# Gadersd/whisper-burn

Hardware: AMD Instinct MI355X
Metric: real-time factor (audio-sec/wall-sec) (higher is better)
Workload: dtype f32; 1 GPU; tiny.en, 30 s of 16 kHz audio per GPU per step, reference windowing (3 windows <= 14.9 s, 3 s overlap), HIP mel + encoder + KV-cached decode, greedy (beam_size 1), max_depth 100; windows=3, beam_size=1, max_depth=100, encoder_gemm_after_the_run=f16x3, parallelism=windows sharded over 1 GPU(s), 1 token all-gather

## Files before the change

### whisper-burn_amd/csrc/decode.h

```cpp
#pragma once
#include <hip/hip_runtime.h>
#include <hip/hip_ext.h>
#include <stdint.h>

#include <algorithm>

#include "kernels.h"
#include "wb_internal.h"

namespace wb {

constexpr int MAX_BEAMS = 8;
constexpr int TOPK_MAX = 8;
constexpr int CA_STRIDE = 66;
constexpr int CA_NCH_MAX = 12;
constexpr int TS_STRIDE = 2 + 2 * TOPK_MAX;
constexpr int GV_CT = 128;
constexpr int GV_CT_LOGITS = 128;
constexpr int KS_MAX = 16;

enum { ST_N = 0, ST_STEP = 1, ST_HDR = 4 };
enum { GC_STEP = 0, GC_NDONE = 1, GC_ALLDONE = 2, GC_BAD = 3, GC_HDR = 4 };
struct StepLayout {
  int S = 0, W = 0;
  int tok = 0, parent = 0, len = 0, win = 0;
  int dead = 0;
  int win_nb = 0, win_slots = 0;
  int total = 0;
};
inline StepLayout make_step_layout(int S, int W) {
  StepLayout l;
  l.S = S; l.W = W;
  l.tok = ST_HDR; l.parent = l.tok + S; l.len = l.parent + S; l.win = l.len + S; l.dead = l.win + S;
  l.win_nb = l.dead + S; l.win_slots = l.win_nb + W; l.total = l.win_slots + W * MAX_BEAMS;
  return l;
}

enum { PRO_PLAIN = 0, PRO_GELU = 1, PRO_ATTN = 2, PRO_LN = 3 };
struct GemvArgs {
  const float* W = nullptr; int ldw = 0;
  int K = 0, N = 0, KS = 1, KSL = 0;
  int pro = PRO_PLAIN;
  const float* src = nullptr; int ld_src = 0;
  const float* pend = nullptr; const float* pbias = nullptr; int KSp = 0;
  float* x_out = nullptr;
  const float* ln_g = nullptr; const float* ln_b = nullptr; float ln_eps = 0.f; int ln_inside = 0;
  int n_head = 0, n_chunks = 0;
  float* P = nullptr;
  float* h_tmp = nullptr;
  const float* mask = nullptr; int use_mask = 0, topk = 0; float* tstats = nullptr;
  const int* st = nullptr; int S = 0;
  int ct = 0;
};

void gemv_plan(int K, int N, int* KS, int* KSL);
int cross_attn_chunk();

void launch_dec_prepare(hipStream_t st, const int* state_host_mapped, int* state_dev, const StepLayout& lay, int n,
                        int* tabs, int Lmax, const float* E, const float* pos, int d, float* x, const int* gctl);
void launch_dec_resolve_ln(hipStream_t st, const int* state, int n_max, const float* x_in, float* x_out,
                           const float* P, int KS, int S, const float* bias, int d, const LayerNormW& ln,
                           int eps_inside_sqrt, float* h);
void launch_dec_gemv(hipStream_t st, const GemvArgs& a, int n_rows_hint, bool stats);
bool dec_logits_two_launches(const GemvArgs& a, int n_rows_hint);
void launch_dec_self_attn(hipStream_t st, const int* state, const StepLayout& lay, int n_max, int n_head,
                          const float* Pqkv, int KS, const float* bqkv, int d, float* Kc, float* Vc, const int* tab,
                          int Lmax, float scale, float* att);
struct CaFuse {
  const float* x_in = nullptr;
  const float* pend = nullptr; int KSp = 0; const float* pbias = nullptr;
  float* x_out = nullptr;
  const float* ln_g = nullptr; const float* ln_b = nullptr; float ln_eps = 0.f; int ln_inside = 0;
  const float* Wq = nullptr;
  const float* Wo = nullptr;
  float* rec = nullptr;
};
bool cross_attn_can_fuse_q(int d);
void launch_dec_cross_attn(hipStream_t st, const int* state, const StepLayout& lay, int n_windows, int n_head,
                           int n_chunks, const float* Pq, int KS, const float* bq, int d, const float* ckv, int ldkv,
                           int koff, const int* win_row0, const int* win_C, float scale, float* ca, int max_nb,
                           const CaFuse* fuse = nullptr);
constexpr int CSF_MAX_D = 1280;
struct CaStreamFuse {
  const float* x_in = nullptr; float* x_out = nullptr;
  const float* pend = nullptr; int KSp = 0; const float* pbias = nullptr;
  const float* ln_g = nullptr; const float* ln_b = nullptr; float ln_eps = 0.f; int ln_inside = 0;
  const float* Wq = nullptr;
};
bool cross_stream_can_fuse(int d);
void launch_dec_cross_attn_stream_fused(hipStream_t st, const int* state, const StepLayout& lay, int n_windows, int n_head,
                                        const float* bq, int d, const float* ckv, int ldkv, int koff, const int* win_row0,
                                        const int* win_C, float scale, float* att, const CaStreamFuse& fz);
void launch_dec_cross_attn_stream(hipStream_t st, const int* state, const StepLayout& lay, int n_windows, int n_head,
                                  const float* Pq, int KS, const float* bq, int d, const float* ckv, int ldkv, int koff,
                                  const int* win_row0, const int* win_C, float scale, float* att);
struct NextPrep {
  float* x = nullptr;
  const float* E = nullptr;
  const float* pos = nullptr;
  int* tabs = nullptr;
  int d = 0;
  int* hflags = nullptr;
};
void launch_dec_topk_merge(hipStream_t st, int* state, int n_max, const float* tstats, int n_tiles, int k,
                           int32_t* out_id, float* out_lp, float* row_stats, const StepLayout& lay, int* gctl, int* gtok,
                           int Lmax, int eot, const NextPrep& nx);
void launch_dec_gelu_fold(hipStream_t st, const int* state, int n_max, const float* P, int KS, int S, int K,
                          const float* bias, float* out);
void launch_dec_attn_combine(hipStream_t st, const int* state, int n_max, const float* ca, int n_head, int n_chunks,
                             float* out);
void launch_dec_topk_rows(hipStream_t st, int* state, int n_max, const float* logits, int V, const float* mask,
                          int use_mask, int k, int32_t* out_id, float* out_lp, float* row_stats, const StepLayout& lay,
                          int* gctl, int* gtok, int Lmax, int eot);
void launch_dec_logprob_row(hipStream_t st, const float* x, int KS, int64_t plane, int V, const float* mask,
                            int use_mask, const float* stats, float* out);

constexpr int BEAM_KB = 2 * TOPK_MAX;
enum { BC_DEPTH = 0, BC_ALLDONE = 1, BC_ERR = 2, BC_NLIVE = 3, BC_HDR = 8 };
struct BeamChainLayout {
  int W = 0, max_depth = 0;
  int nb = 0, done = 0, node = 0, fin = 0, prev_slot = 0, slot_now = 0, lp = 0, nodes = 0, total_ints = 0;
};
inline BeamChainLayout make_beam_layout(int W, int max_depth) {
  BeamChainLayout b;
  b.W = W; b.max_depth = max_depth;
  b.nb = BC_HDR; b.done = b.nb + W; b.node = b.done + W; b.fin = b.node + W * BEAM_KB; b.prev_slot = b.fin + W * BEAM_KB;
  b.slot_now = b.prev_slot + W * BEAM_KB;
  b.lp = (b.slot_now + W * BEAM_KB + 1) & ~1;
  b.nodes = b.lp + 2 * W * BEAM_KB;
  b.total_ints = b.nodes + 2 * (max_depth + 1) * W * BEAM_KB;
  return b;
}
struct BeamChainArgs {
  int* ctl = nullptr; BeamChainLayout bl;
  const int32_t* topk_id = nullptr; const float* topk_lp = nullptr;
  int* state_out = nullptr; StepLayout lay;
  int k = 0, eot = 0, first = 0;
  int V = 0;
  int step_pos = 0;
  int* done_flag_host = nullptr;
  int* tabs = nullptr; int Lmax = 0; const float* E = nullptr; const float* pos = nullptr; int d = 0; float* x = nullptr;
};
void launch_dec_beam_update(hipStream_t st, const BeamChainArgs& a);

struct MlpFusedArgs {
  const int* st = nullptr; int S = 0, d = 0;
  const float* x_in = nullptr; const float* pend = nullptr; int KSp = 0; const float* pbias = nullptr; float* x_out = nullptr;
  int n_head = 0, n_chunks = 0;
  const float* ln_g = nullptr; const float* ln_b = nullptr; float ln_eps = 0.f; int ln_inside = 0;
  const float* W1 = nullptr; int ld1 = 0; const float* b1 = nullptr;
  const float* W2 = nullptr;
  float* P = nullptr;
  unsigned long long* stamps = nullptr;
  int row0 = 0;
  const void* g_x_in = nullptr; const void* g_pend = nullptr; void* g_x_out = nullptr; void* g_P = nullptr;
};
struct AttnFusedArgs {
  const int* st = nullptr; StepLayout lay; int S = 0, d = 0, n_head = 0;
  const float* x_in = nullptr; const float* pend = nullptr; int KSp = 0; const float* pbias = nullptr; float* x_out = nullptr;
  const float* ln_g = nullptr; const float* ln_b = nullptr; float ln_eps = 0.f; int ln_inside = 0;
  const float* Wqkv = nullptr; int ldqkv = 0; const float* bqkv = nullptr; float scale = 0.f;
  float* Kc = nullptr; float* Vc = nullptr; const int* tabs = nullptr; int Lmax = 0;
  const float* Wo = nullptr;
  float* P = nullptr;
  unsigned long long* stamps = nullptr;
  const void* g_x_in = nullptr; const void* g_pend = nullptr; void* g_x_out = nullptr; void* g_P = nullptr;
};
struct CrossFusedArgs {
  const int* st = nullptr; StepLayout lay; int S = 0, d = 0, n_head = 0;
  const float* x_in = nullptr; const float* pend = nullptr; int KSp = 0; const float* pbias = nullptr; float* x_out = nullptr;
  const float* ln_g = nullptr; const float* ln_b = nullptr; float ln_eps = 0.f; int ln_inside = 0;
  const float* Wq = nullptr; const float* bq = nullptr; float scale = 0.f;
  const float* ckv = nullptr; int ldkv = 0, koff = 0;
  const int* win_row0 = nullptr; const int* win_C = nullptr;
  int n_pass = 1;
  const float* Wo = nullptr;
  float* P = nullptr;
  unsigned long long* stamps = nullptr;
  const void* g_x_in = nullptr; const void* g_pend = nullptr; void* g_x_out = nullptr; void* g_P = nullptr;
};
struct SkinnyArgs {
  const float* A = nullptr; int lda = 0;
  const float* B = nullptr; int ldb = 0;
  int M = 0, N = 0, K = 0, ksplit = 1;
  float* P = nullptr; int plane = 0;
  const uint16_t* Bh = nullptr; const uint16_t* Bl = nullptr;
  int* range_flag = nullptr;
  const int* st = nullptr;
};
void launch_split_weight_f16_tiles(hipStream_t st, const float* W, int K, int N, uint16_t* hi, uint16_t* lo);
int skinny_ksplit(int K, int N, int max_ks, int max_rows);
bool skinny_supported(int M, int K, int N);
int launch_dec_skinny_gemm(hipStream_t st, const SkinnyArgs& a);

struct PsLayerArgs { AttnFusedArgs attn; CrossFusedArgs cross; MlpFusedArgs mlp; };
enum { PSR_ATTN = 0, PSR_CROSS = 1, PSR_MLP = 2, PSR_LOGITS = 3, PSR_MERGE = 4, PSR_FINLN = 5 };
struct PsRole { int kind, layer, a, b; };
constexpr int PS_MAX_FORCED = 8;
struct PersistArgs {
  const PsLayerArgs* layers = nullptr;
  const PsRole* roles = nullptr; int n_roles = 0;
  const int* role_off = nullptr;
  int n_logits_roles = 0;
  int n_layer = 0, n_rows = 0, S = 0, d = 0, n_head = 0, nb_mlp = 0;
  int n_pass = 1;
  int* ctl = nullptr;
  int step0 = 0, n_steps = 0;
  int n_forced = 0; int forced[PS_MAX_FORCED] = {0, 0, 0, 0, 0, 0, 0, 0};
  int mask_until_len = 0;
  const void* x_fin = nullptr; const void* P2 = nullptr; const float* b2_last = nullptr;
  void* g_xn = nullptr;
  unsigned tag_base = 0;
  const float* ln_g = nullptr; const float* ln_b = nullptr; float ln_eps = 0.f; int ln_inside = 0;
  const float* Et = nullptr; int vocab_ld = 0, V = 0; const float* mask = nullptr;
  float* tstats = nullptr; int n_tiles = 0;
  int* gctl = nullptr; int* gtok = nullptr; int Lmax = 0, eot = 0;
  const float* E = nullptr; const float* pos = nullptr; void* x0 = nullptr; int* tabs = nullptr;
  int* dead = nullptr;
  unsigned long long* stamps = nullptr;
};
int ps_ctl_ints(int S, int n_layer);
bool dec_persist_supported(int d, int n_rows, int max_keys);
int dec_persist_max_grid(int device, int d, int n_rows, int max_keys);
int launch_dec_persist(hipStream_t st, const PersistArgs& a, int grid);
void launch_ps_seed(hipStream_t st, const float* x, int n, void* gx, unsigned tag);

#if defined(HIPEMU) && !defined(HIPEMU_PROD_GEOMETRY)
constexpr int CROSS_FUSED_MAX_C = 384;
#else
constexpr int CROSS_FUSED_MAX_C = 768;
#endif
constexpr int CROSS_FUSED_MAX_PASSES = 2;
void launch_dec_cross_fused(hipStream_t st, const CrossFusedArgs& a, int n_rows_hint);
bool dec_fused_supported(int d);
int dec_mlp_fused_planes(int d);
void launch_dec_mlp_fused(hipStream_t st, const MlpFusedArgs& a, int n_rows_hint);
void launch_dec_attn_fused(hipStream_t st, const AttnFusedArgs& a, int n_rows_hint);

}
```

### whisper-burn_amd/csrc/decode_chain.cpp

```cpp
#include <climits>
#include <cstring>

#include "decode_step.h"
#include "handoff.h"
#include "switches.h"

using namespace wb;

namespace wb {

static int run_persistent_chain(wb_session* s, int eot, int max_depth, int mask_until_len, const int32_t* forced, int n_forced,
                                int* steps_done, bool* fell_back) {
  *fell_back = false;
  WB_REQUIRE(n_forced >= 0 && n_forced <= PS_MAX_FORCED, WB_ERR_ARG, "persistent decode: %d prompt steps", n_forced);
  const char* inject = sw::persist_inject_fail();
  wb_model* m = s->m;
  const wb_dims& D = m->dims;
  const int d = D.n_text_state, H = D.n_text_head, NL = D.n_text_layer, V = D.n_vocab, S = s->S, W = s->W;
  const StepLayout& L = s->lay;
  hipStream_t st = s->st;
  const int NB = dec_mlp_fused_planes(d);
  const int n_tiles = (V + 127) / 128;
  const size_t pool = (size_t)s->Lmax * S;
  const int ldkv = 2 * d;
  WB_REQUIRE(NB <= 32 && H <= 8, WB_ERR_SHAPE, "persistent decode: more planes than its folds hold");
  WB_TRY(s->ps_gx.ensure_zeroed(((size_t)2 * S + 8) * d * 8, st));
  WB_TRY(s->ps_gpa.ensure_zeroed(((size_t)H * S + 8) * d * 8, st));
  WB_TRY(s->ps_gpc.ensure_zeroed(((size_t)H * S + 8) * d * 8, st));
  WB_TRY(s->ps_gp2.ensure_zeroed(((size_t)NB * S + 8) * d * 8, st));
  WB_TRY(s->ps_gxn.ensure_zeroed(((size_t)S + 8) * d * 8, st));
  if (((s->ps_launches + 1) & 0xffffu) == 0) {
    for (DevMem* b : {&s->ps_gx, &s->ps_gpa, &s->ps_gpc, &s->ps_gp2, &s->ps_gxn}) WB_HIP(hipMemsetAsync(b->p, 0, b->bytes, st));
    s->ps_launches++;
  }
  const unsigned tag_base = ((++s->ps_launches) & 0xffffu) << 16;
  char* gxb[2] = {static_cast<char*>(s->ps_gx.p), static_cast<char*>(s->ps_gx.p) + (size_t)S * d * 8};
  std::vector<PsLayerArgs> la(NL);
  float* xb[2] = {s->x.as<float>(), s->x.as<float>() + (size_t)S * d};
  int xi = 0;
  for (int l = 0; l < NL; l++) {
    const DecBlockW& b = m->dec[l];
    AttnFusedArgs& fa = la[l].attn;
    fa.st = s->state.as<int>(); fa.lay = L; fa.S = S; fa.d = d; fa.n_head = H;
    fa.x_in = xb[xi]; fa.pend = l == 0 ? nullptr : s->P2.as<float>(); fa.KSp = l == 0 ? 0 : NB;
    fa.pbias = l == 0 ? nullptr : m->dec[l - 1].mlp2.b; fa.x_out = xb[xi ^ 1];
    fa.ln_g = b.ln1.g; fa.ln_b = b.ln1.b; fa.ln_eps = b.ln1.eps; fa.ln_inside = m->ln_eps_inside_sqrt;
    fa.Wqkv = b.qkv.w; fa.ldqkv = b.qkv.n; fa.bqkv = b.qkv.b; fa.scale = m->qk_scale;
    fa.Kc = s->kc.as<float>() + (size_t)l * pool * d; fa.Vc = s->vc.as<float>() + (size_t)l * pool * d;
    fa.tabs = s->tabs.as<int>(); fa.Lmax = s->Lmax; fa.Wo = b.out.w; fa.P = s->Pa.as<float>();
    fa.g_x_in = gxb[xi]; fa.g_pend = l == 0 ? nullptr : s->ps_gp2.p; fa.g_x_out = gxb[xi ^ 1]; fa.g_P = s->ps_gpa.p;
    xi ^= 1;
    CrossFusedArgs& ca = la[l].cross;
    ca.st = s->state.as<int>(); ca.lay = L; ca.S = S; ca.d = d; ca.n_head = H;
    ca.x_in = xb[xi]; ca.pend = s->Pa.as<float>(); ca.KSp = H; ca.pbias = b.out.b; ca.x_out = xb[xi ^ 1];
    ca.ln_g = b.ln2.g; ca.ln_b = b.ln2.b; ca.ln_eps = b.ln2.eps; ca.ln_inside = m->ln_eps_inside_sqrt;
    ca.Wq = b.cq.w; ca.bq = b.cq.b; ca.scale = m->qk_scale;
    ca.ckv = s->ckv.as<float>() + (size_t)l * s->enc_rows * 2 * d; ca.ldkv = ldkv; ca.koff = 0;
    ca.win_row0 = s->win_meta.as<int>(); ca.win_C = s->win_meta.as<int>() + W;
    ca.Wo = b.cout.w; ca.P = s->Pc.as<float>();
    ca.n_pass = s->maxC > CROSS_FUSED_MAX_C ? 2 : 1;
    ca.g_x_in = gxb[xi]; ca.g_pend = s->ps_gpa.p; ca.g_x_out = gxb[xi ^ 1]; ca.g_P = s->ps_gpc.p;
    xi ^= 1;
    MlpFusedArgs& ma = la[l].mlp;
    ma.st = s->state.as<int>(); ma.S = S; ma.d = d;
    ma.x_in = xb[xi]; ma.pend = s->Pc.as<float>(); ma.KSp = H; ma.pbias = b.cout.b; ma.x_out = xb[xi ^ 1];
    ma.ln_g = b.ln3.g; ma.ln_b = b.ln3.b; ma.ln_eps = b.ln3.eps; ma.ln_inside = m->ln_eps_inside_sqrt;
    ma.W1 = b.mlp1.w; ma.ld1 = b.mlp1.n; ma.b1 = b.mlp1.b; ma.W2 = b.mlp2.w; ma.P = s->P2.as<float>();
    ma.g_x_in = gxb[xi]; ma.g_pend = s->ps_gpc.p; ma.g_x_out = gxb[xi ^ 1]; ma.g_P = s->ps_gp2.p;
    xi ^= 1;
  }
  std::vector<PsRole> lr;
  for (int l = 0; l < NL; l++) {
    for (int r = 0; r < W; r++) for (int h = 0; h < H; h++) lr.push_back(PsRole{PSR_ATTN, l, h, r});
    for (int r = 0; r < W; r++) for (int h = 0; h < H; h++) lr.push_back(PsRole{PSR_CROSS, l, h, r});
    for (int j = 0; j < NB; j++) lr.push_back(PsRole{PSR_MLP, l, j, 0});
  }
  const int grid = std::max(1, std::min(s->ps_grid, (int)lr.size() + n_tiles + 2 * W));
  std::vector<std::vector<PsRole>> deal(grid);
  for (size_t i = 0; i < lr.size(); i++) deal[i % grid].push_back(lr[i]);
  std::vector<int> cand;
  for (int b = 0; b < grid; b++) {
    bool early = false;
    for (const PsRole& r : deal[b]) early |= r.layer == 0 && (r.kind == PSR_ATTN || r.kind == PSR_CROSS);
    if (!early) cand.push_back(b);
  }
  if ((int)cand.size() * 4 < n_tiles) { cand.clear(); for (int b = 0; b < grid; b++) cand.push_back(b); }
  std::vector<char> is_fin(grid, 0);
  {
    std::vector<int> order(grid);
    for (int b = 0; b < grid; b++) order[b] = b;
    std::stable_sort(order.begin(), order.end(), [&](int x, int y) { return deal[x].size() < deal[y].size(); });
    for (int r = 0; r < W; r++) { deal[order[r % grid]].push_back(PsRole{PSR_FINLN, 0, 0, r}); is_fin[order[r % grid]] = 1; }
  }
  if ((int)cand.size() > 2 * W) cand.erase(std::remove_if(cand.begin(), cand.end(), [&](int b) { return is_fin[b] != 0; }), cand.end());
  std::stable_sort(cand.begin(), cand.end(), [&](int x, int y) { return deal[x].size() < deal[y].size(); });
  const int tpb = (n_tiles + (int)cand.size() - 1) / (int)cand.size();
  const int n_lg = (n_tiles + tpb - 1) / tpb;
  for (int q = 0; q < n_lg; q++)
    deal[cand[q]].push_back(PsRole{PSR_LOGITS, q, q * tpb, std::min(tpb, n_tiles - q * tpb)});
  {
    std::vector<int> order(grid);
    for (int b = 0; b < grid; b++) order[b] = b;
    std::stable_sort(order.begin(), order.end(), [&](int x, int y) { return deal[x].size() < deal[y].size(); });
    for (int r = 0; r < W; r++) deal[order[r % grid]].push_back(PsRole{PSR_MERGE, 0, 0, r});
  }
  std::vector<PsRole> roles;
  std::vector<int> role_off(grid + 1, 0);
  for (int b = 0; b < grid; b++) {
    role_off[b] = (int)roles.size();
    roles.insert(roles.end(), deal[b].begin(), deal[b].end());
  }
  role_off[grid] = (int)roles.size();
  const int n_ctl = ps_ctl_ints(S, NL);
  WB_TRY(s->ps_layers.ensure(la.size() * sizeof(PsLayerArgs)));
  WB_TRY(s->ps_roles.ensure(roles.size() * sizeof(PsRole) + role_off.size() * 4));
  WB_TRY(s->ps_ctl.ensure((size_t)n_ctl * 4));
  WB_TRY(s->ps_dead.ensure((size_t)S * 4));
  WB_TRY(s->ps_tstats.ensure((size_t)S * n_tiles * 2 * 4));
  std::vector<int> ctl0(n_ctl, 0);
  ctl0[HX_STOP] = INT_MAX;
  WB_HIP(hipMemcpyAsync(s->ps_layers.p, la.data(), la.size() * sizeof(PsLayerArgs), hipMemcpyHostToDevice, st));
  WB_HIP(hipMemcpyAsync(s->ps_roles.p, roles.data(), roles.size() * sizeof(PsRole), hipMemcpyHostToDevice, st));
  WB_HIP(hipMemcpyAsync(static_cast<char*>(s->ps_roles.p) + roles.size() * sizeof(PsRole), role_off.data(), role_off.size() * 4,
                        hipMemcpyHostToDevice, st));
  WB_HIP(hipMemcpyAsync(s->ps_ctl.p, ctl0.data(), (size_t)n_ctl * 4, hipMemcpyHostToDevice, st));
  WB_HIP(hipMemsetAsync(s->ps_dead.p, 0, (size_t)S * 4, st));
  PersistArgs a;
  a.layers = s->ps_layers.as<PsLayerArgs>(); a.roles = s->ps_roles.as<PsRole>(); a.n_roles = (int)roles.size();
  a.role_off = reinterpret_cast<const int*>(static_cast<char*>(s->ps_roles.p) + roles.size() * sizeof(PsRole));
  a.n_logits_roles = n_lg;
  a.n_layer = NL; a.n_rows = W; a.S = S; a.d = d; a.n_head = H; a.nb_mlp = NB;
  a.n_pass = s->maxC > CROSS_FUSED_MAX_C ? 2 : 1;
  a.ctl = s->ps_ctl.as<int>(); a.step0 = s->step; a.n_steps = n_forced + max_depth; a.mask_until_len = mask_until_len;
  a.n_forced = n_forced;
  for (int i = 0; i < n_forced; i++) a.forced[i] = forced[i];
  a.g_xn = s->ps_gxn.p;
  a.x_fin = gxb[xi]; a.P2 = s->ps_gp2.p; a.b2_last = m->dec[NL - 1].mlp2.b; a.tag_base = tag_base;
  a.ln_g = m->ln_dec.g; a.ln_b = m->ln_dec.b; a.ln_eps = m->ln_dec.eps; a.ln_inside = m->ln_eps_inside_sqrt;
  a.Et = m->tok_emb_t; a.vocab_ld = m->vocab_ld; a.V = V; a.mask = s->mask.as<float>();
  a.tstats = s->ps_tstats.as<float>(); a.n_tiles = n_tiles;
  a.gctl = s->gctl.as<int>(); a.gtok = s->gtok.as<int>(); a.Lmax = s->Lmax; a.eot = eot;
  a.E = m->tok_emb; a.pos = m->dec_pos; a.x0 = gxb[0]; a.tabs = s->tabs.as<int>(); a.dead = s->ps_dead.as<int>();
  const char* stamps_path = sw::ps_stamps();
  const size_t n_stamps = stamps_path ? (size_t)(n_forced + max_depth) * roles.size() * 8 : 0;
  if (n_stamps) {
    WB_TRY(s->ps_stamps.ensure(n_stamps * 8));
    WB_HIP(hipMemsetAsync(s->ps_stamps.p, 0, n_stamps * 8, st));
    a.stamps = s->ps_stamps.as<unsigned long long>();
  }
  WB_REQUIRE(3 * NL * (n_forced + max_depth + 1) + 4 < 0x10000, WB_ERR_SHAPE,
             "persistent decode: %d layers x %d steps do not fit the 16-bit granule tags", NL, max_depth);
  launch_dec_prepare(st, reinterpret_cast<const int*>(s->host_block_dev), s->state.as<int>(), L, W, s->tabs.as<int>(),
                     s->Lmax, m->tok_emb, m->dec_pos, d, s->x.as<float>(), s->gctl.as<int>());
  launch_ps_seed(st, s->x.as<float>(), W * d, gxb[0], tag_base + 1u);
  WB_HIP(hipStreamSynchronize(st));
  hipEvent_t e0 = nullptr, e1 = nullptr;
  prof_tag(KC_PERSIST, 0.0);
  const bool timed = prof_take_events(&e0, &e1);
  if (timed) WB_HIP(hipEventRecord(e0, st));
  const bool refused = (inject && !strcmp(inject, "launch")) || launch_dec_persist(st, a, grid) != 0;
  if (timed) WB_HIP(hipEventRecord(e1, st));
  if (refused) {
    (void)hipGetLastError();
    s->ps_grid = 0;
    *fell_back = true;
    *steps_done = 0;
    return WB_OK;
  }
  std::vector<int> ctl(n_ctl);
  WB_HIP(hipMemcpyAsync(ctl.data(), s->ps_ctl.p, (size_t)n_ctl * 4, hipMemcpyDeviceToHost, st));
  int gstep = 0;
  WB_HIP(hipMemcpyAsync(&gstep, s->gctl.as<int>() + GC_STEP, 4, hipMemcpyDeviceToHost, st));
  WB_HIP(hipStreamSynchronize(st));
  if (ctl[HX_ERR] != 0 && gstep == s->step) {
    s->ps_grid = 0;
    *fell_back = true;
    *steps_done = 0;
    return WB_OK;
  }
  WB_REQUIRE(ctl[HX_ERR] == 0, WB_ERR_HIP, "persistent decode: a wait gave up (counter %d) at step %d", ctl[HX_ERR] - 1, gstep);
  if (n_stamps) {
    std::vector<unsigned long long> hs(n_stamps);
    WB_HIP(hipMemcpy(hs.data(), s->ps_stamps.p, n_stamps * 8, hipMemcpyDeviceToHost));
    if (FILE* f = fopen(stamps_path, "wb")) {
      const int hdr[4] = {n_forced + max_depth, (int)roles.size(), grid, 8};
      fwrite(hdr, 4, 4, f);
      std::vector<int> kinds(roles.size());
      for (size_t i = 0; i < roles.size(); i++)
        kinds[i] = roles[i].kind | ((roles[i].kind <= PSR_MLP ? roles[i].layer : 0) << 8) |
                   ((roles[i].kind == PSR_LOGITS ? 0 : roles[i].b) << 16);
      fwrite(kinds.data(), 4, kinds.size(), f);
      fwrite(hs.data(), 8, hs.size(), f);
      fclose(f);
    }
  }
  *steps_done = std::max(0, std::min(n_forced + max_depth, gstep - s->step));
  return WB_OK;
}

int session_greedy_chain(wb_session* s, const int32_t* prompt, int eot, int max_depth, int mask_until_len, int prompt_len,
                         int32_t* out_tokens, int32_t row_stride, int32_t* out_lens) {
  wb_model* m = s->m;
  const int S = s->S, W = s->W;
  WB_REQUIRE(S == W, WB_ERR_STATE, "chained greedy decode needs max_beams == 1");
  WB_REQUIRE(prompt && prompt_len >= 1, WB_ERR_ARG, "chained greedy decode: empty prompt");
  WB_REQUIRE(s->step == 0 || (s->prev_n == W && s->step == prompt_len - 1), WB_ERR_STATE,
             "chained greedy decode: the session is neither fresh nor prefilled");
  const int n_forced_max = prompt_len - 1;
  auto host_prefill = [&]() -> int {
    std::vector<int32_t> tok(W), par(W), win(W);
    for (int t = s->step; t < prompt_len - 1; t++) {
      for (int w = 0; w < W; w++) { tok[w] = prompt[t]; par[w] = t == 0 ? -1 : w; win[w] = w; }
      WB_TRY(wb_session_step(s, tok.data(), par.data(), win.data(), W, 0, 0, nullptr, nullptr));
    }
    return WB_OK;
  };
  WB_REQUIRE(s->has_mask || mask_until_len < prompt_len || max_depth == 0, WB_ERR_STATE,
             "wb_session_decode: special mask not set");
  const int asked_depth = max_depth;
  max_depth = std::min(max_depth, s->Lmax - (prompt_len - 1));
  WB_HIP(hipSetDevice(m->device));
  hipStream_t st = s->st;
  const size_t ctl_ints = GC_HDR + 3 * (size_t)S;
  WB_TRY(s->gctl.ensure(ctl_ints * 4));
  WB_TRY(s->gtok.ensure(((size_t)S * s->Lmax + 1) * 4));
  std::vector<int> ctl(ctl_ints, 0);
  auto seed_ctl = [&]() -> int {
    std::fill(ctl.begin(), ctl.end(), 0);
    ctl[GC_STEP] = s->step;
    for (int i = 0; i < W; i++) ctl[GC_HDR + i] = prompt[s->step];
    WB_HIP(hipMemcpyAsync(s->gctl.p, ctl.data(), ctl_ints * 4, hipMemcpyHostToDevice, st));
    WB_HIP(hipStreamSynchronize(st));
    return WB_OK;
  };
  const StepPlan plan = plan_step(s, W, false);
  const int n_launch = plan.n_launch;
  const bool fuse_ln = plan.fuse_ln;
  const int chunk = 16;
  int depth = 0;
  bool persist = plan.persist && max_depth > 0;
  if (persist) {
    if (s->ps_grid < 0) s->ps_grid = dec_persist_max_grid(m->device, m->dims.n_text_state, W, s->maxC);
    persist = s->ps_grid > 0;
  }
  int n_forced = 0;
  if (persist && sw::persist_prefill() && s->step == 0 && n_forced_max <= PS_MAX_FORCED && s->has_mask) n_forced = n_forced_max;
  if (n_forced == 0) WB_TRY(host_prefill());
  WB_TRY(seed_ctl());
  ScopedTimer tm(st, 3);
  if (persist) {
    bool fell_back = false;
    WB_TRY(run_persistent_chain(s, eot, max_depth, mask_until_len, prompt + s->step + 1, n_forced, &depth, &fell_back));
    if (fell_back) {
      persist = false;
      depth = 0;
      WB_TRY(host_prefill());
      WB_TRY(seed_ctl());
      n_forced = 0;
    } else {
      if (profile().on) profile().ms[4] += depth;
      depth -= n_forced;
      s->step += n_forced;
      s->prev_n = W;
      s->prev_win.resize(W);
      for (int w = 0; w < W; w++) s->prev_win[w] = w;
    }
  }
  if (!persist) {
  if (fuse_ln)
    launch_dec_prepare(st, reinterpret_cast<const int*>(s->host_block_dev), s->state.as<int>(), s->lay, n_launch,
                       s->tabs.as<int>(), s->Lmax, m->tok_emb, m->dec_pos, m->dims.n_text_state, s->x.as<float>(),
                       s->gctl.as<int>());
  const bool speculate = fuse_ln && sw::speculate();
  if (speculate && !s->st2) {
    WB_HIP(hipStreamCreateWithFlags(&s->st2, hipStreamNonBlocking));
    WB_HIP(hipEventCreateWithFlags(&s->ev_seg, hipEventDisableTiming));
  }
  auto enqueue_segment = [&](int* enq) -> int {
    int n = 0;
    while (depth + n < max_depth && n < chunk) {
      const int d0 = depth + n;
      const int use_mask = (prompt_len + d0) <= mask_until_len ? 1 : 0;
      const int run = (!use_mask && max_depth - d0 >= chunk) ? chunk : 1;
      StepCall call;
      call.k = 1; call.use_mask = use_mask; call.chained = true; call.eot = eot; call.reps = run;
      WB_TRY(launch_step(s, plan, call));
      if (profile().on) profile().ms[4] += run;
      n += run;
    }
    *enq = n;
    return WB_OK;
  };
  auto read_flags = [&](bool behind_event) -> int {
    if (behind_event) {
      WB_HIP(hipStreamWaitEvent(s->st2, s->ev_seg, 0));
      WB_HIP(hipMemcpyAsync(ctl.data(), s->gctl.p, ctl_ints * 4, hipMemcpyDeviceToHost, s->st2));
      WB_HIP(hipStreamSynchronize(s->st2));
    } else {
      WB_HIP(hipMemcpyAsync(ctl.data(), s->gctl.p, ctl_ints * 4, hipMemcpyDeviceToHost, st));
      WB_HIP(hipStreamSynchronize(st));
    }
    return WB_OK;
  };
  auto all_done = [&]() {
    bool d = true;
    for (int i = 0; i < W; i++) d = d && ctl[GC_HDR + S + i] != 0;
    return d;
  };
  const bool poll = fuse_ln && sw::poll() && !profile().on;
  volatile int* hfl = reinterpret_cast<volatile int*>(s->host_block + s->chain_flags_off);
  if (poll) for (int i = 0; i < 2 * S; i++) hfl[i] = 0;
  auto wait_flags = [&](int want_step, bool* done) -> int {
    for (long spins = 0;; spins++) {
      bool ready = true;
      for (int i = 0; i < W && ready; i++) ready = hfl[2 * i] >= want_step;
      if (ready) break;
      bool fin = true;
      for (int i = 0; i < W && fin; i++) fin = hfl[2 * i + 1] != 0;
      if (fin) break;
      if ((spins & 0xfff) == 0xfff) {
        const hipError_t q = hipStreamQuery(st);
        if (q == hipSuccess) {
          bool r2 = true;
          for (int i = 0; i < W && r2; i++) r2 = hfl[2 * i] >= want_step;
          if (r2) break;
          bool all = true;
          for (int i = 0; i < W; i++) all = all && hfl[2 * i + 1] != 0;
          if (all) break;
          set_error("chained decode: the device stopped at step %d of %d", (int)hfl[0], want_step);
          return WB_ERR_HIP;
        }
        if (q != hipErrorNotReady) { set_error("chained decode: %s", hipGetErrorString(q)); return WB_ERR_HIP; }
      }
    }
    __atomic_thread_fence(__ATOMIC_ACQUIRE);
    bool all = true;
    for (int i = 0; i < W; i++) all = all && hfl[2 * i + 1] != 0;
    *done = all;
    return WB_OK;
  };
  if (!speculate) {
    while (depth < max_depth) {
      int n = 0;
      WB_TRY(enqueue_segment(&n));
      depth += n;
      if (poll) {
        bool done = false;
        WB_TRY(wait_flags(s->step + depth, &done));
        if (done) break;
      } else {
        WB_TRY(read_flags(false));
        if (all_done()) break;
      }
    }
  } else {
    int n_cur = 0;
    WB_TRY(enqueue_segment(&n_cur));
    depth += n_cur;
    while (true) {
      WB_HIP(hipEventRecord(s->ev_seg, st));
      int n_next = 0;
      if (depth < max_depth) { WB_TRY(enqueue_segment(&n_next)); depth += n_next; }
      WB_TRY(read_flags(true));
      if (all_done() || n_next == 0) break;
    }
    WB_HIP(hipStreamSynchronize(st));
  }
  }
  tm.stop();
  std::vector<int> toks((size_t)S * s->Lmax + 1);
  WB_HIP(hipMemcpyAsync(ctl.data(), s->gctl.p, ctl_ints * 4, hipMemcpyDeviceToHost, st));
  WB_HIP(hipMemcpyAsync(toks.data(), s->gtok.p, toks.size() * 4, hipMemcpyDeviceToHost, st));
  WB_HIP(hipStreamSynchronize(st));
  tm.collect();
  WB_TRY(dec_split_check(s));
  WB_REQUIRE(ctl[GC_BAD] == 0, WB_ERR_STATE, "a decode step produced a row without a finite log-prob (NaN logits: non-finite "
             "weights or activations); its window was ended on <|endoftext|> on the device and the rows of this call are invalid");
  for (int w = 0; w < W; w++) {
    int len = ctl[GC_HDR + 2 * S + w];
    if (len < prompt_len) len = prompt_len;
    len = std::min(len, prompt_len + max_depth);
    WB_REQUIRE(len <= row_stride, WB_ERR_ARG, "row_stride too small");
    for (int p = prompt_len; p < len; p++) out_tokens[(size_t)w * row_stride + p] = toks[(size_t)w * s->Lmax + p];
    out_lens[w] = len;
  }
  if (profile().on && !persist && s->prof_cls_cross >= 0 && s->prof_cls_self >= 0) {
    const int dm = m->dims.n_text_state, NL = m->dims.n_text_layer;
    double dead_ckv = 0, dead_self = 0;
    for (int w = 0; w < W; w++) {
      const int live = std::max(0, std::min(out_lens[w] - prompt_len, depth));
      for (int t = live; t < depth; t++) { dead_ckv += 8.0 * s->C[w] * dm; dead_self += 8.0 * (s->step + t + 1) * dm; }
    }
    prof_adjust_bytes(s->prof_cls_cross, -(double)NL * dead_ckv);
    prof_adjust_bytes(s->prof_cls_self, -(double)NL * dead_self);
  }
  if (profile().on && persist) {
    const double dm = m->dims.n_text_state, NL = m->dims.n_text_layer;
    double bytes = (double)(depth + n_forced) * 4.0 * NL * 14.0 * dm * dm + (double)depth * 4.0 * (double)m->dims.n_vocab * dm;
    for (int w = 0; w < W; w++)
      for (int t = 0; t < n_forced; t++) bytes += NL * (8.0 * s->C[w] * dm + 8.0 * (t + 1) * dm);
    for (int w = 0; w < W; w++) {
      const int live = std::max(0, std::min(out_lens[w] - prompt_len, depth));
      for (int t = 0; t < live; t++) bytes += NL * (8.0 * s->C[w] * dm + 8.0 * (s->step + t + 1) * dm);
    }
    prof_adjust_bytes(KC_PERSIST, bytes);
  }
  s->prof_step_off = 0;
  s->step += depth;
  s->prev_len.assign(W, s->step);
  s->last_had_logits = 0;
  if (max_depth < asked_depth)
    for (int w = 0; w < W; w++)
      WB_REQUIRE(ctl[GC_HDR + S + w] != 0, WB_ERR_SHAPE, "Token sequence length %d must not exceed %d.", s->Lmax + 1,
                 s->Lmax);
  return WB_OK;
}
}
```

### whisper-burn_amd/csrc/decode_fused.hip

```cpp
#include <hip/hip_runtime.h>

#include <cstdlib>

#include "decode.h"
#include "decode_fused_bodies.h"
#include "switches.h"
#include "wave_ops.h"

namespace wb {
namespace {

using namespace fused;

template <int MR, int DPL, bool REC>
__global__ __launch_bounds__(512) void dec_mlp_fused_kernel(MlpFusedArgs a) {
  if (blockIdx.y > 0) {
    const int r0 = blockIdx.y * MR;
    const int64_t sh = (int64_t)r0 * a.d;
    a.row0 = r0; a.x_in += sh; a.x_out += sh; a.P += sh;
    if (a.pend) a.pend += sh;
  }
  dec_mlp_body<MR, DPL, REC, false>(a, blockIdx.x, PsStep());
}
template <int DPL>
__global__ __launch_bounds__(512) void dec_attn_fused_kernel(AttnFusedArgs a) {
  dec_attn_body<DPL, false>(a, blockIdx.x, blockIdx.y, PsStep());
}
template <int DPL, int NP>
__global__ __launch_bounds__(512) void dec_cross_fused_kernel(CrossFusedArgs a) {
  dec_cross_body<DPL, false, NP>(a, blockIdx.x, blockIdx.y, PsStep());
}


typedef float mm_f32x4 __attribute__((ext_vector_type(4)));
template <int DPL>
__global__ __launch_bounds__(512) void dec_mlp16_mfma_kernel(MlpFusedArgs a) {
  constexpr int MR = 16, d = 64 * DPL, HS = 64, NT = 512;
  constexpr int KW = d / 8;
  constexpr int NL1 = KW / 4, NL2 = HS / 4;
  __shared__ __attribute__((aligned(16))) float xT[d * MR];
  __shared__ __attribute__((aligned(16))) float red[8][MR][HS];
  __shared__ __attribute__((aligned(16))) float hT[HS * MR];
  const int tid = threadIdx.x, lane = tid & 63, wave = tid >> 6;
  const int jblk = blockIdx.x, j0 = jblk * HS;
  const int krow = lane >> 4, cq = lane & 15;
  const int n_rows = min(MR, a.st[ST_N]);
  float4 w1[NL1], w2[NL2];
  {
    const float* p1 = a.W1 + (int64_t)(wave * KW + krow) * a.ld1 + j0 + 4 * cq;
#pragma unroll
    for (int t = 0; t < NL1; t++) w1[t] = *reinterpret_cast<const float4*>(p1 + (int64_t)(4 * t) * a.ld1);
    const int strip = wave < d / 64 ? wave : 0;
    const float* p2 = a.W2 + (int64_t)(j0 + krow) * d + strip * 64 + 4 * cq;
#pragma unroll
    for (int t = 0; t < NL2; t++) w2[t] = *reinterpret_cast<const float4*>(p2 + (int64_t)(4 * t) * d);
  }
  if (n_rows <= 0) return;
#pragma unroll 1
  for (int r = wave; r < MR; r += 8) {
    if (r >= n_rows) {
      for (int c = lane; c < d; c += 64) xT[c * MR + r] = 0.f;
      continue;
    }
    float gv[DPL], bv[DPL], v[DPL];
    const float* xr = a.x_in + (int64_t)r * d;
#pragma unroll
    for (int i = 0; i < DPL; i++) { gv[i] = a.ln_g[lane + 64 * i]; bv[i] = a.ln_b[lane + 64 * i]; v[i] = xr[lane + 64 * i]; }
    if (a.KSp > 0) {
      float acc[DPL];
#pragma unroll
      for (int i = 0; i < DPL; i++) acc[i] = a.pbias[lane + 64 * i];
      const float* pp = a.pend + (int64_t)r * d;
      const int64_t plane = (int64_t)a.S * d;
      constexpr int CH = 8;
      for (int sp = 0; sp < a.KSp; sp += CH) {
        float t[CH][DPL];
#pragma unroll
        for (int j = 0; j < CH; j++) {
          const float* pj = pp + (int64_t)min(sp + j, a.KSp - 1) * plane;
#pragma unroll
          for (int i = 0; i < DPL; i++) t[j][i] = pj[lane + 64 * i];
        }
#pragma unroll
        for (int j = 0; j < CH; j++) {
          const bool live = sp + j < a.KSp;
#pragma unroll
          for (int i = 0; i < DPL; i++) acc[i] += live ? t[j][i] : 0.f;
        }
      }
#pragma unroll
      for (int i = 0; i < DPL; i++) v[i] = v[i] + acc[i];
    }
    float sm = 0.f;
#pragma unroll
    for (int i = 0; i < DPL; i++) { sm += v[i]; if (jblk == 0) a.x_out[(int64_t)r * d + lane + 64 * i] = v[i]; }
    const float mean = wave_sum(sm) / (float)d;
    float q = 0.f;
#pragma unroll
    for (int i = 0; i < DPL; i++) { const float t = v[i] - mean; q += t * t; }
    const float var = wave_sum(q) / (float)d;
    const float denom = a.ln_inside ? sqrtf(var + a.ln_eps) : (sqrtf(var) + a.ln_eps);
#pragma unroll
    for (int i = 0; i < DPL; i++) xT[(lane + 64 * i) * MR + r] = (v[i] - mean) / denom * gv[i] + bv[i];
  }
  __syncthreads();
  {
    mm_f32x4 acc[4];
#pragma unroll
    for (int c = 0; c < 4; c++) acc[c] = mm_f32x4{0.f, 0.f, 0.f, 0.f};
    const float* ap = xT + (wave * KW) * MR + lane;
#pragma unroll
    for (int t = 0; t < NL1; t++) {
      const float av = ap[(4 * t) * MR];
      acc[0] = __builtin_amdgcn_mfma_f32_16x16x4f32(av, w1[t].x, acc[0], 0, 0, 0);
      acc[1] = __builtin_amdgcn_mfma_f32_16x16x4f32(av, w1[t].y, acc[1], 0, 0, 0);
      acc[2] = __builtin_amdgcn_mfma_f32_16x16x4f32(av, w1[t].z, acc[2], 0, 0, 0);
      acc[3] = __builtin_amdgcn_mfma_f32_16x16x4f32(av, w1[t].w, acc[3], 0, 0, 0);
    }
#pragma unroll
    for (int i = 0; i < 4; i++)
      *reinterpret_cast<float4*>(&red[wave][4 * krow + i][4 * cq]) = make_float4(acc[0][i], acc[1][i], acc[2][i], acc[3][i]);
  }
  __syncthreads();
#pragma unroll
  for (int e = tid; e < MR * HS; e += NT) {
    const int r = e / HS, c = e - r * HS;
    float hsum = a.b1[j0 + c];
#pragma unroll
    for (int w8 = 0; w8 < 8; w8++) hsum += red[w8][r][c];
    hT[c * MR + r] = r < n_rows ? gelu_erf_f(hsum) : 0.f;
  }
  __syncthreads();
  if (wave < d / 64) {
    mm_f32x4 acc[4];
#pragma unroll
    for (int c = 0; c < 4; c++) acc[c] = mm_f32x4{0.f, 0.f, 0.f, 0.f};
#pragma unroll
    for (int t = 0; t < NL2; t++) {
      const float av = hT[(4 * t) * MR + lane];
      acc[0] = __builtin_amdgcn_mfma_f32_16x16x4f32(av, w2[t].x, acc[0], 0, 0, 0);
      acc[1] = __builtin_amdgcn_mfma_f32_16x16x4f32(av, w2[t].y, acc[1], 0, 0, 0);
      acc[2] = __builtin_amdgcn_mfma_f32_16x16x4f32(av, w2[t].z, acc[2], 0, 0, 0);
      acc[3] = __builtin_amdgcn_mfma_f32_16x16x4f32(av, w2[t].w, acc[3], 0, 0, 0);
    }
#pragma unroll
    for (int i = 0; i < 4; i++) {
      const int r = 4 * krow + i;
      if (r < n_rows)
        *reinterpret_cast<float4*>(&a.P[((int64_t)jblk * a.S + r) * d + wave * 64 + 4 * cq]) =
            make_float4(acc[0][i], acc[1][i], acc[2][i], acc[3][i]);
    }
  }
}

}

bool dec_fused_supported(int d) { return d == 128 || d == 384 || d == 512; }
int dec_mlp_fused_planes(int d) { return 4 * d / 64; }

void launch_dec_mlp_fused(hipStream_t st, const MlpFusedArgs& a, int n_rows_hint) {
  if (sw::mlp16_mfma() && n_rows_hint > 8 && n_rows_hint <= 16 && a.n_chunks == 0 && a.row0 == 0) {
    const dim3 grid16(4 * a.d / 64), block16(512);
    if (a.d == 128) WB_KLAUNCH((dec_mlp16_mfma_kernel<2>), grid16, block16, 0, st, a);
    else if (a.d == 384) WB_KLAUNCH((dec_mlp16_mfma_kernel<6>), grid16, block16, 0, st, a);
    else WB_KLAUNCH((dec_mlp16_mfma_kernel<8>), grid16, block16, 0, st, a);
    return;
  }
  const dim3 grid(4 * a.d / 64, n_rows_hint > 8 ? (n_rows_hint + 7) / 8 : 1), block(512);
#define WB_MLP(MR_, DPL_)                                                                          \
  do {                                                                                             \
    if (a.n_chunks > 0) WB_KLAUNCH((dec_mlp_fused_kernel<MR_, DPL_, true>), grid, block, 0, st, a); \
    else WB_KLAUNCH((dec_mlp_fused_kernel<MR_, DPL_, false>), grid, block, 0, st, a);               \
  } while (0)
  if (n_rows_hint <= 4) {
    if (a.d == 128) WB_MLP(4, 2); else if (a.d == 384) WB_MLP(4, 6); else WB_MLP(4, 8);
  } else {
    if (a.d == 128) WB_MLP(8, 2); else if (a.d == 384) WB_MLP(8, 6); else WB_MLP(8, 8);
  }
#undef WB_MLP
}

void launch_dec_cross_fused(hipStream_t st, const CrossFusedArgs& a, int n_rows_hint) {
  const dim3 grid(a.n_head <= 8 ? 8 : a.n_head, n_rows_hint), block(512);
  if (a.n_pass <= 1) {
    if (a.d == 128) WB_KLAUNCH((dec_cross_fused_kernel<2, 1>), grid, block, 0, st, a);
    else if (a.d == 384) WB_KLAUNCH((dec_cross_fused_kernel<6, 1>), grid, block, 0, st, a);
    else WB_KLAUNCH((dec_cross_fused_kernel<8, 1>), grid, block, 0, st, a);
  } else {
    if (a.d == 128) WB_KLAUNCH((dec_cross_fused_kernel<2, 2>), grid, block, 0, st, a);
    else if (a.d == 384) WB_KLAUNCH((dec_cross_fused_kernel<6, 2>), grid, block, 0, st, a);
    else WB_KLAUNCH((dec_cross_fused_kernel<8, 2>), grid, block, 0, st, a);
  }
}

void launch_dec_attn_fused(hipStream_t st, const AttnFusedArgs& a, int n_rows_hint) {
  const dim3 grid(a.n_head <= 8 ? 8 : a.n_head, n_rows_hint), block(512);
  if (a.d == 128) WB_KLAUNCH((dec_attn_fused_kernel<2>), grid, block, 0, st, a);
  else if (a.d == 384) WB_KLAUNCH((dec_attn_fused_kernel<6>), grid, block, 0, st, a);
  else WB_KLAUNCH((dec_attn_fused_kernel<8>), grid, block, 0, st, a);
}

}
```

### whisper-burn_amd/csrc/decode_fused_bodies.h

```cpp
#pragma once
#include <hip/hip_runtime.h>

#include "decode.h"
#include "handoff.h"
#include "wave_ops.h"

namespace wb {
namespace fused {

struct PsStep {
  const unsigned* ctr = nullptr; unsigned target = 0; int ctr_index = 0;
  const int* ctl = nullptr;
  int step = 0;
  int n_rows = 0;
  const int* dead = nullptr;
  int* lds_flag = nullptr;
  unsigned long long* stamp = nullptr;
  int n_ctr = 1;
  unsigned tag_in = 0, tag_out = 0;
  bool known_dead = false;
  mutable bool saw_dead = false;
};
constexpr int PS_STAMPS = 8;
__device__ __forceinline__ void ps_stamp(const PsStep& ps, int k) {
#ifdef WB_EXP_FINE
  if (k == 4 || k == 5) return;
#endif
  if (ps.stamp && threadIdx.x == 0) ps.stamp[k] = wall_clock64();
}
__device__ __forceinline__ void ps_stamp_fine(const PsStep& ps, int k) {
#ifdef WB_EXP_FINE
  if (ps.stamp && threadIdx.x == 0) ps.stamp[k] = wall_clock64();
#endif
}
__device__ __forceinline__ bool ps_wait(const PsStep& ps) {
  const bool ok = ps.n_ctr > 1 ? hx_wait_same(ps.ctr, ps.target, ps.n_ctr, ps.ctl, ps.step, ps.ctr_index, ps.lds_flag)
                               : hx_wait(ps.ctr, ps.target, ps.ctl, ps.step, ps.ctr_index, ps.lds_flag);
  ps_stamp(ps, 1);
  return ok;
}
__device__ __forceinline__ bool ps_sweep_retry(unsigned& sweeps, const PsStep& ps) {
  if ((sweeps & 31u) == 31u &&
      (__hip_atomic_load(ps.ctl + HX_STOP, __ATOMIC_RELAXED, __HIP_MEMORY_SCOPE_AGENT) <= ps.step ||
       __hip_atomic_load(ps.ctl + HX_ERR, __ATOMIC_RELAXED, __HIP_MEMORY_SCOPE_AGENT) != 0)) return true;
  if (++sweeps > HX_SWEEP_LIMIT) {
    __hip_atomic_store(const_cast<int*>(ps.ctl) + HX_ERR, 5000 + ps.ctr_index, __ATOMIC_RELAXED, __HIP_MEMORY_SCOPE_AGENT);
    return true;
  }
  __builtin_amdgcn_s_sleep(1);
  return false;
}
__device__ __forceinline__ bool ps_sweeps_ok(const PsStep& ps) { return *ps.lds_flag != 0; }
template <int UNITS>
__device__ __forceinline__ void ps_nap() {
#if !defined(WB_PS_DRY) || defined(WB_PS_DRY_NAPS)
#ifndef WB_PS_NAP_ADJ
#define WB_PS_NAP_ADJ 0
#endif
#pragma unroll
  for (int i = 0; i < UNITS + (WB_PS_NAP_ADJ); i++) __builtin_amdgcn_s_sleep(64);
#endif
}

#ifdef WB_STAMPS
#define WB_STAMP_DECL __shared__ unsigned long long stamp_buf[16]
#define WB_STAMP(i) do { if (threadIdx.x == 0 && blockIdx.x == 0 && blockIdx.y == 0) stamp_buf[i] = wall_clock64(); } while (0)
#define WB_STAMP_FLUSH(a, n) do { if (threadIdx.x == 0 && blockIdx.x == 0 && blockIdx.y == 0 && (a).stamps) for (int _i = 0; _i < (n); _i++) (a).stamps[_i] = stamp_buf[_i]; } while (0)
#else
#define WB_STAMP_DECL
#define WB_STAMP(i) do {} while (0)
#define WB_STAMP_FLUSH(a, n) do {} while (0)
#endif

constexpr int FD_MAX = 512;
constexpr int FA_MAXPOS = 448;

__device__ __forceinline__ float gelu_erf_f(float x) {
  return 0.5f * x * (1.0f + erff(x * 0.70710678118654752440f));
}

template <int DPL>
__device__ __forceinline__ void fold_ln_row(const float* __restrict__ x_in, const float* __restrict__ pend, int KSp,
                                            int64_t plane, const float* __restrict__ pbias, float* __restrict__ x_out,
                                            const float* __restrict__ g, const float* __restrict__ b, float eps,
                                            int eps_inside, int d, int row, int lane, float* __restrict__ out) {
  int co[DPL];
#pragma unroll
  for (int i = 0; i < DPL; i++) co[i] = lane + (64 * i < d ? 64 * i : 0);
  float gv[DPL], bv[DPL], v[DPL];
  const float* xr = x_in + (int64_t)row * d;
#pragma unroll
  for (int i = 0; i < DPL; i++) { gv[i] = g[co[i]]; bv[i] = b[co[i]]; v[i] = xr[co[i]]; }
  if (KSp > 0) {
    float acc[DPL];
#pragma unroll
    for (int i = 0; i < DPL; i++) acc[i] = pbias[co[i]];
    const float* pp = pend + (int64_t)row * d;
    constexpr int CH = DPL <= 6 ? 8 : 4;
    for (int sp = 0; sp < KSp; sp += CH) {
      float t[CH][DPL];
#pragma unroll
      for (int j = 0; j < CH; j++) {
        const float* pj = pp + (int64_t)min(sp + j, KSp - 1) * plane;
#pragma unroll
        for (int i = 0; i < DPL; i++) t[j][i] = pj[co[i]];
      }
#pragma unroll
      for (int j = 0; j < CH; j++) {
        const bool live = sp + j < KSp;
#pragma unroll
        for (int i = 0; i < DPL; i++) acc[i] += live ? t[j][i] : 0.f;
      }
    }
#pragma unroll
    for (int i = 0; i < DPL; i++) v[i] = v[i] + acc[i];
  }
  float s = 0.f;
#pragma unroll
  for (int i = 0; i < DPL; i++) {
    if (64 * i < d) { s += v[i]; if (x_out) x_out[(int64_t)row * d + co[i]] = v[i]; }
  }
  const float mean = wave_sum(s) / (float)d;
  float q = 0.f;
#pragma unroll
  for (int i = 0; i < DPL; i++) {
    if (64 * i < d) { const float t = v[i] - mean; q += t * t; }
  }
  const float var = wave_sum(q) / (float)d;
  const float denom = eps_inside ? sqrtf(var + eps) : (sqrtf(var) + eps);
#pragma unroll
  for (int i = 0; i < DPL; i++) {
    const int c = lane + 64 * i;
    if (c < d) out[c] = (v[i] - mean) / denom * gv[i] + bv[i];
  }
}

template <int NT, int MR, int EPT, int PCH>
__device__ __forceinline__ void fold_rows(const float* __restrict__ x_in, const float* __restrict__ pend, int KSp,
                                          int64_t plane, const float* __restrict__ pbias, int d, int tid,
                                          float (&v)[EPT]) {
  int off[EPT], col[EPT];
#pragma unroll
  for (int i = 0; i < EPT; i++) {
    int e = tid + NT * i;
    if (e >= MR * d) e = tid;
    off[i] = e; col[i] = e % d;
  }
#pragma unroll
  for (int i = 0; i < EPT; i++) v[i] = x_in[off[i]];
  if (KSp > 0) {
    float acc[EPT];
#pragma unroll
    for (int i = 0; i < EPT; i++) acc[i] = pbias[col[i]];
    for (int sp = 0; sp < KSp; sp += PCH) {
      float t[PCH][EPT];
#pragma unroll
      for (int j = 0; j < PCH; j++) {
        const float* pj = pend + (int64_t)min(sp + j, KSp - 1) * plane;
#pragma unroll
        for (int i = 0; i < EPT; i++) t[j][i] = pj[off[i]];
      }
#pragma unroll
      for (int j = 0; j < PCH; j++) {
        const bool live = sp + j < KSp;
#pragma unroll
        for (int i = 0; i < EPT; i++) acc[i] += live ? t[j][i] : 0.f;
      }
    }
#pragma unroll
    for (int i = 0; i < EPT; i++) v[i] = v[i] + acc[i];
  }
}

template <int DPL>
__device__ __forceinline__ void ln_row_lds(float* __restrict__ row, int d, int lane, const float (&gv)[DPL],
                                           const float (&bv)[DPL], float eps, int eps_inside) {
  float v[DPL];
  float s = 0.f;
#pragma unroll
  for (int i = 0; i < DPL; i++) { v[i] = row[lane + 64 * i]; s += v[i]; }
  const float mean = wave_sum(s) / (float)d;
  float q = 0.f;
#pragma unroll
  for (int i = 0; i < DPL; i++) { const float t = v[i] - mean; q += t * t; }
  const float var = wave_sum(q) / (float)d;
  const float denom = eps_inside ? sqrtf(var + eps) : (sqrtf(var) + eps);
#pragma unroll
  for (int i = 0; i < DPL; i++) row[lane + 64 * i] = (v[i] - mean) / denom * gv[i] + bv[i];
}

template <int DPL>
__device__ __forceinline__ void ln_stats_lds(const float* __restrict__ row, int d, int lane, float eps, int eps_inside,
                                             float& mean, float& denom) {
  float v[DPL];
  float s = 0.f;
#pragma unroll
  for (int i = 0; i < DPL; i++) { v[i] = row[lane + 64 * i]; s += v[i]; }
  mean = wave_sum(s) / (float)d;
  float q = 0.f;
#pragma unroll
  for (int i = 0; i < DPL; i++) { const float t = v[i] - mean; q += t * t; }
  const float var = wave_sum(q) / (float)d;
  denom = eps_inside ? sqrtf(var + eps) : (sqrtf(var) + eps);
}
__device__ __forceinline__ float lane_get(float v, int src) { return __shfl(v, src, 64); }

template <int MR, int DPL, bool REC, bool PS>
__device__ __forceinline__ bool dec_mlp_body(const MlpFusedArgs& a, const int jblk, const PsStep& ps) {
  constexpr int HS = 64, NT = 512;
  constexpr int d = 64 * DPL;
  constexpr int CF = d / 4;
  constexpr int G = CF <= 32 ? 8 : 4;
  constexpr int RPG = HS / G;
  constexpr int EPT = (MR * d + NT - 1) / NT;
  constexpr int PCH = EPT <= 3 ? 8 : EPT <= 6 ? 6 : 3;
  __shared__ __attribute__((aligned(16))) float hs[MR][d];
  __shared__ __attribute__((aligned(16))) float red[8][MR][HS];
  __shared__ __attribute__((aligned(16))) float hid[MR][HS];
  __shared__ __attribute__((aligned(16))) float obuf[(G - 1) * MR * d];
  __shared__ float mlb[REC ? MR : 1][48][2];
  __shared__ float coef[REC ? MR : 1][48];
  WB_STAMP_DECL;
  WB_STAMP(0);
  const int tid = role_tid<PS>(), lane = tid & 63, wave = tid >> 6;
  const int j0 = jblk * HS;
  const int rg = tid >> 4, c4 = (tid & 15) * 4;
  float xv_fold[EPT];
  constexpr int NW1 = d / 32;
  float4 w1[NW1];
  const int cf = tid % CF, jg = tid / CF;
  const bool p2 = jg < G;
  const int jb = (p2 ? jg : 0) * RPG;
  float4 w2[RPG];
  constexpr int NOWN = 4 * NW1;
  const int own_col = 4 * wave + (lane & 3) + 32 * ((lane < NOWN ? lane : 0) >> 2);
  float g_own = 0.f, b_own = 0.f;
  float b1v;
  int deadm = 0;
  {
    int off[EPT], col[EPT];
#pragma unroll
    for (int i = 0; i < EPT; i++) {
      int e = tid + NT * i;
      if (e >= MR * d) e = tid;
      off[i] = e; col[i] = e % d;
    }
    float acc0[EPT];
    constexpr bool rec = REC;
    const int64_t plane = rec ? (int64_t)a.S * (d + 2) : (int64_t)a.S * d;
    int poff[EPT];
#pragma unroll
    for (int i = 0; i < EPT; i++) poff[i] = rec ? (off[i] / d) * (d + 2) + 2 + col[i] : off[i];
    constexpr int PCHR = EPT <= 3 ? 18 : EPT <= 4 ? 16 : EPT <= 6 ? 12 : 8;
    constexpr int PC = REC ? PCHR : PCH;
    float t[PC][EPT];
    const int npl = a.KSp;
    const int ch = rec ? PCHR : PCH;
    auto load_weights = [&]() {
      g_own = gld(a.ln_g + own_col); b_own = gld(a.ln_b + own_col);
      b1v = gld(a.b1 + j0 + (tid & 63));
      {
        const float* wp = a.W1 + (int64_t)rg * a.ld1 + j0 + c4;
#pragma unroll
        for (int i = 0; i < NW1; i++) w1[i] = ld_w4(wp + (int64_t)(32 * i) * a.ld1);
      }
      {
        const float* wp = a.W2 + (int64_t)(j0 + jb) * d + cf * 4;
#pragma unroll
        for (int i = 0; i < RPG; i++) w2[i] = ld_w4(wp + (int64_t)i * d);
      }
    };
    if constexpr (PS) {
#if !defined(WB_PS_DRY)
      load_weights();
#endif
      if (!ps_wait(ps)) return false;
#pragma unroll
      for (int r = 0; r < MR; r++)
        if (r >= ps.n_rows || ld_i<true>(ps.dead + min(r, ps.n_rows - 1)) != 0) deadm |= 1 << r;
      const Buf16 xgb(a.g_x_in), pgb(a.g_pend);
      const int iplane = a.S * d;
      ps_nap<3>();
      bool rdead[EPT];
#pragma unroll
      for (int i = 0; i < EPT; i++) { rdead[i] = ((deadm >> (off[i] / d)) & 1) != 0; acc0[i] = gld(a.pbias + col[i]); xv_fold[i] = 0.f; }
      constexpr int GP = EPT <= 3 ? 8 : 4;
      unsigned sweeps = 0;
      bool bad = false;
      for (int sp = 0; sp < npl && !bad; sp += GP) {
        Gran gx[EPT], g[GP][EPT];
#pragma unroll
        for (int i = 0; i < EPT; i++) {
          gx[i] = Gran{0u, 0.f};
#pragma unroll
          for (int j = 0; j < GP; j++) g[j][i] = Gran{0u, 0.f};
        }
        for (;;) {
          if (sp == 0) {
#pragma unroll
            for (int i = 0; i < EPT; i++)
              if (!rdead[i] && gx[i].tag != ps.tag_in) gx[i] = ld_gran(xgb, (uint32_t)off[i], 0u);
          }
#pragma unroll
          for (int j = 0; j < GP; j++)
#pragma unroll
            for (int i = 0; i < EPT; i++)
              if (!rdead[i] && sp + j < npl && g[j][i].tag != ps.tag_in)
                g[j][i] = ld_gran(pgb, (uint32_t)off[i], (uint32_t)((sp + j) * iplane));
          bool ok = true;
#pragma unroll
          for (int i = 0; i < EPT; i++) {
            if (sp == 0) ok &= rdead[i] || gx[i].tag == ps.tag_in;
#pragma unroll
            for (int j = 0; j < GP; j++) ok &= rdead[i] || sp + j >= npl || g[j][i].tag == ps.tag_in;
          }
          if (ok) {
#pragma unroll
            for (int i = 0; i < EPT; i++) {
              if (sp == 0) xv_fold[i] = gx[i].v;
#pragma unroll
              for (int j = 0; j < GP; j++) acc0[i] += (sp + j < npl) ? g[j][i].v : 0.f;
            }
            break;
          }
          if (ps_sweep_retry(sweeps, ps)) { *ps.lds_flag = 0; bad = true; break; }
        }
      }
#pragma unroll
      for (int i = 0; i < EPT; i++) {
        xv_fold[i] = rdead[i] ? 0.f : xv_fold[i] + acc0[i];
        const int e = tid + NT * i;
        if (e < MR * d) (&hs[0][0])[e] = xv_fold[i];
      }
    } else {
#pragma unroll
    for (int i = 0; i < EPT; i++) { xv_fold[i] = a.x_in[off[i]]; acc0[i] = npl > 0 ? gld(a.pbias + col[i]) : 0.f; }
    float mlv0 = -1.0e30f, mlv1 = 0.f;
    if (rec && tid < MR * npl) {
      const float* rp = a.pend + (int64_t)(tid % npl) * plane + (int64_t)(tid / npl) * (d + 2);
      mlv0 = rp[0]; mlv1 = rp[1];
    }
    if (npl > 0) {
#pragma unroll
      for (int j = 0; j < PC; j++)
        if (j < ch) {
#pragma unroll
          for (int i = 0; i < EPT; i++) t[j][i] = a.pend[(int64_t)min(j, npl - 1) * plane + poff[i]];
        }
    }
    load_weights();
    if constexpr (REC) {
      if (tid < MR * npl) { mlb[tid / npl][tid % npl][0] = mlv0; mlb[tid / npl][tid % npl][1] = mlv1; }
      __syncthreads();
      if (tid < MR * a.n_head) {
        const int r = tid / a.n_head, hh = tid % a.n_head;
        float M = -1.0e30f;
        for (int c = 0; c < a.n_chunks; c++) M = fmaxf(M, mlb[r][hh * a.n_chunks + c][0]);
        float den = 0.f;
        for (int c = 0; c < a.n_chunks; c++) den += expf(mlb[r][hh * a.n_chunks + c][0] - M) * mlb[r][hh * a.n_chunks + c][1];
        for (int c = 0; c < a.n_chunks; c++)
          coef[r][hh * a.n_chunks + c] = den > 0.f ? expf(mlb[r][hh * a.n_chunks + c][0] - M) / den : 0.f;
      }
      __syncthreads();
    }
    if (npl > 0) {
      int rowi[EPT];
#pragma unroll
      for (int i = 0; i < EPT; i++) rowi[i] = off[i] / d;
      for (int sp = 0; sp < npl; sp += ch) {
        if (sp > 0) {
#pragma unroll
          for (int j = 0; j < PC; j++)
            if (j < ch) {
#pragma unroll
              for (int i = 0; i < EPT; i++) t[j][i] = a.pend[(int64_t)min(sp + j, npl - 1) * plane + poff[i]];
            }
        }
#pragma unroll
        for (int j = 0; j < PC; j++)
          if (j < ch) {
#pragma unroll
            for (int i = 0; i < EPT; i++) {
              const bool live = sp + j < npl;
              float wgt = 1.f;
              if constexpr (REC) wgt = coef[rowi[i]][min(sp + j, npl - 1)];
              acc0[i] += live ? wgt * t[j][i] : 0.f;
            }
          }
      }
#pragma unroll
      for (int i = 0; i < EPT; i++) xv_fold[i] += acc0[i];
    }
#pragma unroll
    for (int i = 0; i < EPT; i++) {
      const int e = tid + NT * i;
      if (e < MR * d) (&hs[0][0])[e] = xv_fold[i];
    }
    }
  }
  int n_rows;
  if constexpr (PS) n_rows = ps.n_rows; else n_rows = min(MR, a.st[ST_N] - a.row0);
  if (n_rows <= 0) return true;
  WB_STAMP(1);
  __syncthreads();
  if constexpr (PS) { if (!ps_sweeps_ok(ps)) return false; }
#if defined(WB_PS_DRY)
  if constexpr (PS) {
    if (jg == 0) {
      const Buf16 pgo(a.g_P);
#pragma unroll
      for (int r = 0; r < MR; r++)
        if (r < n_rows && !((deadm >> r) & 1)) st_gran4(pgo, (uint32_t)((jblk * a.S + r) * d + cf * 4), ps.tag_out, make_float4(0.f, 0.f, 0.f, 0.f));
    }
    if (jblk == 0) {
      const Buf16 xgo(a.g_x_out);
#pragma unroll
      for (int i = 0; i < EPT; i++) {
        const int e = tid + NT * i;
        if (e < n_rows * d && !((deadm >> (e / d)) & 1)) st_gran(xgo, (uint32_t)e, ps.tag_out, xv_fold[i]);
      }
    }
    return true;
  }
#endif
  float xn_own[MR];
#pragma unroll
  for (int r = 0; r < MR; r++) {
    xn_own[r] = 0.f;
    bool skip = r >= n_rows;
    if constexpr (PS) skip = skip || ((deadm >> r) & 1);
    if (skip) continue;
    float mean, denom;
    ln_stats_lds<DPL>(hs[r], d, lane, a.ln_eps, a.ln_inside, mean, denom);
    xn_own[r] = (hs[r][own_col] - mean) / denom * g_own + b_own;
  }
  WB_STAMP(2);
  float acc[MR][4];
#pragma unroll
  for (int r = 0; r < MR; r++) { acc[r][0] = acc[r][1] = acc[r][2] = acc[r][3] = 0.f; }
  {
    const int q4 = lane >> 4;
#pragma unroll
    for (int r = 0; r < MR; r++) {
      bool skip = r >= n_rows;
      if constexpr (PS) skip = skip || ((deadm >> r) & 1);
      if (skip) continue;
#pragma unroll
      for (int i = 0; i < NW1; i++) {
        const float xv = lane_get(xn_own[r], 4 * i + q4);
        acc[r][0] += xv * w1[i].x; acc[r][1] += xv * w1[i].y; acc[r][2] += xv * w1[i].z; acc[r][3] += xv * w1[i].w;
      }
    }
  }
#pragma unroll
  for (int r = 0; r < MR; r++)
#pragma unroll
    for (int c = 0; c < 4; c++) { acc[r][c] = xor16_sum(acc[r][c]); acc[r][c] = xor32_sum(acc[r][c]); }
  if (lane < 16) {
#pragma unroll
    for (int r = 0; r < MR; r++)
      *reinterpret_cast<float4*>(&red[wave][r][c4]) = make_float4(acc[r][0], acc[r][1], acc[r][2], acc[r][3]);
  }
  __syncthreads();
  if (tid < MR * HS) {
    const int r = tid >> 6, c = tid & 63;
    float v = 0.f;
#pragma unroll
    for (int w8 = 0; w8 < 8; w8++) v += red[w8][r][c];
    hid[r][c] = gelu_erf_f(v + b1v);
  }
  __syncthreads();
  WB_STAMP(3);
  float o[MR][4];
#pragma unroll
  for (int r = 0; r < MR; r++) { o[r][0] = o[r][1] = o[r][2] = o[r][3] = 0.f; }
  if constexpr (PS) {
#pragma unroll
    for (int r = 0; r < MR; r++) {
      if ((deadm >> r) & 1) continue;
#pragma unroll
      for (int i = 0; i < RPG; i++) {
        const float hv = hid[r][jb + i];
        o[r][0] += hv * w2[i].x; o[r][1] += hv * w2[i].y; o[r][2] += hv * w2[i].z; o[r][3] += hv * w2[i].w;
      }
    }
  } else {
#pragma unroll
  for (int i = 0; i < RPG; i++) {
#pragma unroll
    for (int r = 0; r < MR; r++) {
      const float hv = hid[r][jb + i];
      o[r][0] += hv * w2[i].x; o[r][1] += hv * w2[i].y; o[r][2] += hv * w2[i].z; o[r][3] += hv * w2[i].w;
    }
  }
  }
  if (p2 && jg > 0) {
#pragma unroll
    for (int r = 0; r < MR; r++)
      *reinterpret_cast<float4*>(&obuf[((jg - 1) * MR + r) * d + cf * 4]) = make_float4(o[r][0], o[r][1], o[r][2], o[r][3]);
  }
  __syncthreads();
  if (jg == 0) {
#pragma unroll
    for (int g2 = 1; g2 < G; g2++) {
#pragma unroll
      for (int r = 0; r < MR; r++) {
        const float4 t = *reinterpret_cast<const float4*>(&obuf[((g2 - 1) * MR + r) * d + cf * 4]);
        o[r][0] += t.x; o[r][1] += t.y; o[r][2] += t.z; o[r][3] += t.w;
      }
    }
    if constexpr (PS) {
      const Buf16 pgo(a.g_P);
#pragma unroll
      for (int r = 0; r < MR; r++)
        if (r < n_rows && !((deadm >> r) & 1))
          st_gran4(pgo, (uint32_t)((jblk * a.S + r) * d + cf * 4), ps.tag_out, make_float4(o[r][0], o[r][1], o[r][2], o[r][3]));
    } else {
#pragma unroll
      for (int r = 0; r < MR; r++)
        if (r < n_rows)
          *reinterpret_cast<float4*>(&a.P[((int64_t)jblk * a.S + r) * d + cf * 4]) = make_float4(o[r][0], o[r][1], o[r][2], o[r][3]);
    }
  }
  if (jblk == 0) {
    if constexpr (PS) {
      const Buf16 xgo(a.g_x_out);
#pragma unroll
      for (int i = 0; i < EPT; i++) {
        const int e = tid + NT * i;
        if (e < n_rows * d && !((deadm >> (e / d)) & 1)) st_gran(xgo, (uint32_t)e, ps.tag_out, xv_fold[i]);
      }
    } else {
#pragma unroll
      for (int i = 0; i < EPT; i++) {
        const int e = tid + NT * i;
        if (e < n_rows * d) a.x_out[e] = xv_fold[i];
      }
    }
  }
  WB_STAMP(4);
  WB_STAMP_FLUSH(a, 5);
  return true;
}

template <int DPL, bool PS>
__device__ __forceinline__ bool dec_attn_body(const AttnFusedArgs& a, const int h, const int r, const PsStep& ps) {
  constexpr int NT = 512;
  constexpr int d = 64 * DPL;
  constexpr int KW = d / 8;
  constexpr int RK = DPL >= 6 ? 8 : 16;
  constexpr int NIT = KW / RK;
  constexpr int CF = d / 4;
  constexpr int G = CF <= 32 ? 8 : 4;
  constexpr int RPG = 64 / G;
  constexpr int RED = (8 * 192 > (G - 1) * d) ? 8 * 192 : (G - 1) * d;
  constexpr int PT = 128, PSL = PT * 16 / NT;
  __shared__ __attribute__((aligned(16))) float hs[d];
  __shared__ __attribute__((aligned(16))) float red[RED];
  __shared__ __attribute__((aligned(16))) float qkv[192];
  __shared__ int tbs[FA_MAXPOS];
  __shared__ float sc[FA_MAXPOS];
  __shared__ __attribute__((aligned(16))) float part[32][64];
  __shared__ __attribute__((aligned(16))) float att[64];
  WB_STAMP_DECL;
  WB_STAMP(0);
  const int tid = role_tid<PS>(), lane = tid & 63, wave = tid >> 6;
  if (h >= a.n_head) return true;
  int n_rows, len, step_par, dead;
  if constexpr (PS) { n_rows = ps.n_rows; len = ps.step + 1; step_par = 0; dead = 0; }
  else {
    n_rows = a.st[ST_N]; len = a.st[a.lay.len + r]; step_par = a.st[ST_STEP] & 1;
    dead = a.st[a.lay.dead + r];
  }
  const int seg = lane >> 4, c4 = (lane & 15) * 4;
  const bool seg_ok = seg < 3;
  const float* wq = a.Wqkv + (int64_t)(wave * KW) * a.ldqkv + (seg_ok ? seg : 0) * d + h * 64 + c4;
  float4 wr[2][RK];
  auto load_round = [&](float4 (&w)[RK], int it) {
#pragma unroll
    for (int j = 0; j < RK; j++) w[j] = ld_w4(wq + (int64_t)(RK * it + j) * a.ldqkv);
  };
  float xfold;
  const int own_col = wave * KW + (lane < KW ? lane : 0);
  float g_own = 0.f, b_own = 0.f;
  float qbias = 0.f;
  const int npast = len - 1;
  const int rg = tid >> 4, pq4 = (tid & 15) * 4;
  const int* tb = a.tabs + (size_t)step_par * a.lay.S * a.Lmax + r * a.Lmax;
  auto slot_of = [&](int p) { if constexpr (PS) return p * a.lay.S + r; else return tb[p]; };
  int slot_new = 0;
  const Buf16 kbuf(a.Kc), vbuf(a.Vc);
  float4 kc[PSL], vc[PSL];
  auto load_cache_tile = [&]() {
    int slot[PSL];
#pragma unroll
    for (int i = 0; i < PSL; i++) slot[i] = slot_of(rg + 32 * i < npast ? rg + 32 * i : 0);
    slot_new = slot_of(npast);
    if constexpr (!PS) {
      if (npast > PT)
        for (int p = tid; p < npast; p += NT) tbs[p] = tb[p];
    }
#pragma unroll
    for (int i = 0; i < PSL; i++) kc[i] = ld_f4<PS>(a.Kc, kbuf, (uint32_t)(slot[i] * d + h * 64 + pq4));
#pragma unroll
    for (int i = 0; i < PSL; i++) vc[i] = ld_f4<PS>(a.Vc, vbuf, (uint32_t)(slot[i] * d + h * 64 + pq4));
  };
  {
    const int c = tid < d ? tid : 0;
    const float* pp = a.pend + (int64_t)r * d + c;
    const int64_t plane = (int64_t)a.S * d;
    auto load_weights = [&]() {
      g_own = gld(a.ln_g + own_col); b_own = gld(a.ln_b + own_col);
      load_round(wr[0], 0);
      if (NIT > 1) load_round(wr[1], 1);
      if constexpr (PS) { if (tid < 192) qbias = gld(a.bqkv + (tid >> 6) * d + h * 64 + (tid & 63)); }
    };
    if constexpr (PS) {
#if !defined(WB_PS_DRY)
      if (!ps.known_dead) {
        load_weights();
        load_cache_tile();
      }
#endif
      if (!ps_wait(ps)) return false;
      dead = ps.known_dead ? 1 : ld_i<true>(ps.dead + r);
      if (r >= n_rows || dead) { ps.saw_dead = true; return true; }
      const Buf16 xgb(a.g_x_in), pgb(a.g_pend);
      const uint32_t pvo = (uint32_t)(r * d + c);
      const int iplane = a.S * d;
      if (a.KSp > 0) ps_nap<2>();
      constexpr int FP = 4 * DPL;
      float v = 0.f, accp = a.KSp > 0 ? gld(a.pbias + c) : 0.f;
      unsigned sweeps = 0;
      Gran gx{0u, 0.f}, g[FP];
#pragma unroll
      for (int j = 0; j < FP; j++) g[j] = Gran{0u, 0.f};
      for (;;) {
        if (gx.tag != ps.tag_in) gx = ld_gran(xgb, pvo, 0u);
        if (a.KSp > 0) {
#pragma unroll
          for (int j = 0; j < FP; j++)
            if (j < a.KSp && g[j].tag != ps.tag_in) g[j] = ld_gran(pgb, pvo, (uint32_t)(j * iplane));
        }
        bool ok = gx.tag == ps.tag_in;
        if (a.KSp > 0) {
#pragma unroll
          for (int j = 0; j < FP; j++) ok &= (j >= a.KSp) || g[j].tag == ps.tag_in;
        }
        if (ok) {
          v = gx.v;
          if (a.KSp > 0) {
#pragma unroll
            for (int j = 0; j < FP; j++) accp += (j < a.KSp) ? g[j].v : 0.f;
            v += accp;
          }
          break;
        }
        if (ps_sweep_retry(sweeps, ps)) { *ps.lds_flag = 0; break; }
      }
      xfold = v;
      if (tid < d) hs[tid] = v;
    } else {
    float v = a.x_in[(int64_t)r * d + c];
    constexpr int FP = 32;
    float t[FP];
    float accp = 0.f;
    if (a.KSp > 0) {
      accp = gld(a.pbias + c);
#pragma unroll
      for (int j = 0; j < FP; j++) t[j] = pp[(int64_t)min(j, a.KSp - 1) * plane];
    }
    load_weights();
    if (r >= n_rows || dead) return true;
    if (a.KSp > 0) {
#pragma unroll
      for (int j = 0; j < FP; j++) accp += (j < a.KSp) ? t[j] : 0.f;
      for (int sp = FP; sp < a.KSp; sp += FP) {
#pragma unroll
        for (int j = 0; j < FP; j++) t[j] = pp[(int64_t)min(sp + j, a.KSp - 1) * plane];
#pragma unroll
        for (int j = 0; j < FP; j++) accp += (sp + j < a.KSp) ? t[j] : 0.f;
      }
      v += accp;
    }
    xfold = v;
    if (tid < d) hs[tid] = v;
    }
  }
  if constexpr (!PS) qbias = tid < 192 ? a.bqkv[(tid >> 6) * d + h * 64 + (tid & 63)] : 0.f;
  if constexpr (!PS) load_cache_tile();
  WB_STAMP(1);
  if constexpr (PS) ps_stamp(ps, 2);
  __syncthreads();
  if constexpr (PS) { if (!ps_sweeps_ok(ps)) return false; }
#if defined(WB_PS_DRY)
  if constexpr (PS) {
    if (tid < d / 4) { const Buf16 pgo(a.g_P); st_gran4(pgo, (uint32_t)((h * a.S + r) * d + tid * 4), ps.tag_out, make_float4(0.f, 0.f, 0.f, 0.f)); }
    if (h == 0 && tid < d) { const Buf16 xgo(a.g_x_out); st_gran(xgo, (uint32_t)(r * d + tid), ps.tag_out, xfold); }
    return true;
  }
#endif
  float xn_own;
  {
    float mean, denom;
    ln_stats_lds<DPL>(hs, d, lane, a.ln_eps, a.ln_inside, mean, denom);
    xn_own = (hs[own_col] - mean) / denom * g_own + b_own;
  }
  if constexpr (PS) ps_stamp_fine(ps, 4);
  WB_STAMP(2);
  float acc[4] = {0.f, 0.f, 0.f, 0.f};
#pragma unroll 1
  for (int it = 0; it < NIT; it += 2) {
#pragma unroll
    for (int b = 0; b < 2; b++) {
      if (it + b < NIT) {
        const int kb = RK * (it + b);
#pragma unroll
        for (int j = 0; j < RK; j++) {
          const float xv = __int_as_float(__builtin_amdgcn_readlane(__float_as_int(xn_own), kb + j));
          acc[0] += xv * wr[b][j].x; acc[1] += xv * wr[b][j].y; acc[2] += xv * wr[b][j].z; acc[3] += xv * wr[b][j].w;
        }
        if (it + b + 2 < NIT) load_round(wr[b], it + b + 2);
      }
    }
  }
  WB_STAMP(3);
  if constexpr (PS) ps_stamp(ps, 3);
  __syncthreads();
  const int cf = tid % CF, jg = tid / CF;
  const bool p5 = jg < G;
  const int jb = (p5 ? jg : 0) * RPG;
  float4 wo[RPG];
  {
    const float* wp = a.Wo + (int64_t)(h * 64 + jb) * d + cf * 4;
#pragma unroll
    for (int i = 0; i < RPG; i++) wo[i] = ld_w4(wp + (int64_t)i * d);
  }
  if (seg_ok) *reinterpret_cast<float4*>(&red[wave * 192 + seg * 64 + c4]) = make_float4(acc[0], acc[1], acc[2], acc[3]);
  __syncthreads();
  if (tid < 192) {
    float v = 0.f;
#pragma unroll
    for (int w8 = 0; w8 < 8; w8++) v += red[w8 * 192 + tid];
    v += qbias;
    if (tid < 128) v *= a.scale;
    qkv[tid] = v;
  }
  __syncthreads();
  if constexpr (PS) ps_stamp_fine(ps, 5);
  WB_STAMP(4);
  {
    const float4 q4 = *reinterpret_cast<const float4*>(&qkv[pq4]);
    auto row_dot = [&](const float4& k4) {
      float s = q4.x * k4.x + q4.y * k4.y + q4.z * k4.z + q4.w * k4.w;
      s += dpp_f<DPP_QUAD_XOR1, 0xF>(0.f, s);
      s += dpp_f<DPP_QUAD_XOR2, 0xF>(0.f, s);
      s += dpp_f<DPP_ROW_HALF_MIRROR, 0xF>(0.f, s);
      s += dpp_f<DPP_ROW_MIRROR, 0xF>(0.f, s);
      return s;
    };
#pragma unroll
    for (int i = 0; i < PSL; i++) {
      const int p = rg + 32 * i;
      const float s = row_dot(kc[i]);
      if ((tid & 15) == 0 && p < npast) sc[p] = s;
    }
    for (int t0 = PT; t0 < npast; t0 += PT) {
      float4 kt[PSL];
#pragma unroll
      for (int i = 0; i < PSL; i++) {
        const int p = min(t0 + rg + 32 * i, npast - 1);
        int sl;
        if constexpr (PS) sl = p * a.lay.S + r; else sl = tbs[p];
        kt[i] = ld_f4<PS>(a.Kc, kbuf, (uint32_t)(sl * d + h * 64 + pq4));
      }
#pragma unroll
      for (int i = 0; i < PSL; i++) {
        const int p = t0 + rg + 32 * i;
        const float s = row_dot(kt[i]);
        if ((tid & 15) == 0 && p < npast) sc[p] = s;
      }
    }
    if (wave == 7) {
      const float s = wave_sum(qkv[lane] * qkv[64 + lane]);
      if (lane == 0) sc[npast] = s;
    }
  }
  __syncthreads();
  WB_STAMP(5);
  if constexpr (PS) ps_stamp(ps, 4);
  float m = -INFINITY;
  for (int p = lane; p < len; p += 64) m = fmaxf(m, sc[p]);
  m = wave_max(m);
  float l = 0.f;
  for (int p = lane; p < len; p += 64) l += expf(sc[p] - m);
  l = wave_sum(l);
  {
    float4 o = make_float4(0.f, 0.f, 0.f, 0.f);
#pragma unroll
    for (int i = 0; i < PSL; i++) {
      const int p = rg + 32 * i;
      const float pk = p < npast ? expf(sc[p] - m) : 0.f;
      o.x += pk * vc[i].x; o.y += pk * vc[i].y; o.z += pk * vc[i].z; o.w += pk * vc[i].w;
    }
    for (int t0 = PT; t0 < npast; t0 += PT) {
      float4 vt[PSL];
#pragma unroll
      for (int i = 0; i < PSL; i++) {
        const int p = min(t0 + rg + 32 * i, npast - 1);
        int sl;
        if constexpr (PS) sl = p * a.lay.S + r; else sl = tbs[p];
        vt[i] = ld_f4<PS>(a.Vc, vbuf, (uint32_t)(sl * d + h * 64 + pq4));
      }
#pragma unroll
      for (int i = 0; i < PSL; i++) {
        const int p = t0 + rg + 32 * i;
        const float pk = p < npast ? expf(sc[p] - m) : 0.f;
        o.x += pk * vt[i].x; o.y += pk * vt[i].y; o.z += pk * vt[i].z; o.w += pk * vt[i].w;
      }
    }
    *reinterpret_cast<float4*>(&part[rg][pq4]) = o;
  }
  __syncthreads();
  if (tid < 64) {
    float v = 0.f;
#pragma unroll
    for (int g2 = 0; g2 < 32; g2++) v += part[g2][tid];
    v += expf(sc[npast] - m) * qkv[128 + tid];
    att[tid] = v / l;
  }
  __syncthreads();
  WB_STAMP(6);
  if constexpr (PS) ps_stamp(ps, 5);
  float ov[4] = {0.f, 0.f, 0.f, 0.f};
#pragma unroll
  for (int i = 0; i < RPG; i++) {
    const float av = att[jb + i];
    ov[0] += av * wo[i].x; ov[1] += av * wo[i].y; ov[2] += av * wo[i].z; ov[3] += av * wo[i].w;
  }
  if (p5 && jg > 0)
    *reinterpret_cast<float4*>(&red[(jg - 1) * d + cf * 4]) = make_float4(ov[0], ov[1], ov[2], ov[3]);
  __syncthreads();
  if (jg == 0) {
#pragma unroll
    for (int g2 = 1; g2 < G; g2++) {
      const float4 t = *reinterpret_cast<const float4*>(&red[(g2 - 1) * d + cf * 4]);
      ov[0] += t.x; ov[1] += t.y; ov[2] += t.z; ov[3] += t.w;
    }
    if constexpr (PS) {
      const Buf16 pgo(a.g_P);
      st_gran4(pgo, (uint32_t)((h * a.S + r) * d + cf * 4), ps.tag_out, make_float4(ov[0], ov[1], ov[2], ov[3]));
    } else {
      *reinterpret_cast<float4*>(&a.P[((int64_t)h * a.S + r) * d + cf * 4]) = make_float4(ov[0], ov[1], ov[2], ov[3]);
    }
  }
  if (tid >= 64 && tid < 192) {
    float* dst = (tid < 128 ? a.Kc : a.Vc) + (int64_t)slot_new * d + h * 64 + (tid & 63);
    st_f<PS>(dst, qkv[tid]);
  }
  if (h == 0 && tid < d) {
    if constexpr (PS) { const Buf16 xgo(a.g_x_out); st_gran(xgo, (uint32_t)(r * d + tid), ps.tag_out, xfold); }
    else a.x_out[(int64_t)r * d + tid] = xfold;
  }
  WB_STAMP(7);
  WB_STAMP_FLUSH(a, 8);
  return true;
}

template <int DPL, bool PS, int NP = 1>
__device__ __forceinline__ bool dec_cross_body(const CrossFusedArgs& a, const int h, const int r, const PsStep& ps) {
  constexpr int NT = 512;
  constexpr int PASS_C = CROSS_FUSED_MAX_C, CMAX = NP * PASS_C;
  constexpr int d = 64 * DPL;
  constexpr int NWQ = d / 32;
  constexpr int CF = d / 4;
  constexpr int G = CF <= 32 ? 8 : 4;
  constexpr int RPG = 64 / G;
  constexpr int KT = 128, NTILE = CROSS_FUSED_MAX_C / KT, SL = KT * 16 / NT;
  static_assert(CROSS_FUSED_MAX_C % KT == 0 && SL * NT == KT * 16, "tile geometry");
  __shared__ __attribute__((aligned(16))) float hs[d];
  __shared__ __attribute__((aligned(16))) float red[8][64];
  __shared__ __attribute__((aligned(16))) float qv[64];
  __shared__ float sc[CMAX];
  __shared__ float pbuf[CMAX];
  __shared__ __attribute__((aligned(16))) float part[32][64];
  __shared__ __attribute__((aligned(16))) float att[64];
  __shared__ __attribute__((aligned(16))) float obuf[(G - 1) * d];
  const int tid = role_tid<PS>(), lane = tid & 63, wave = tid >> 6;
  if (h >= a.n_head) return true;
  int n_live, w_row, dead;
  if constexpr (PS) { n_live = ps.n_rows; w_row = r; dead = 0; }
  else {
    n_live = a.st[ST_N]; w_row = a.st[a.lay.win + r];
    dead = a.st[a.lay.dead + r];
  }
  const int wi8 = min(lane & 7, a.lay.W - 1);
  const int vC8 = gld(a.win_C + wi8), vR8 = gld(a.win_row0 + wi8);
  float xfold;
  const int rg = tid >> 4, c4 = (tid & 15) * 4;
  constexpr int NOWN = 4 * NWQ;
  const int own_col = 4 * wave + (lane & 3) + 32 * ((lane < NOWN ? lane : 0) >> 2);
  float g_own = 0.f, b_own = 0.f;
  float4 wqr[NWQ];
  float4 kv[NTILE][SL];
  const float* Kh; const float* Vh; int C;
  float qbias = 0.f;
  auto load_weights = [&]() {
    g_own = gld(a.ln_g + own_col); b_own = gld(a.ln_b + own_col);
    if constexpr (PS) { if (tid < 64) qbias = gld(a.bq + h * 64 + tid); }
    {
      const float* wp = a.Wq + (int64_t)rg * d + h * 64 + c4;
#pragma unroll
      for (int i = 0; i < NWQ; i++) wqr[i] = ld_w4(wp + (int64_t)(32 * i) * d);
    }
  };
  auto load_keys = [&]() {
    int C_w, row0_w;
    {
      const int ws = __builtin_amdgcn_readfirstlane(w_row);
      if (ws < 8) { C_w = __builtin_amdgcn_readlane(vC8, ws); row0_w = __builtin_amdgcn_readlane(vR8, ws); }
      else { C_w = gld(a.win_C + ws); row0_w = gld(a.win_row0 + ws); }
    }
    C = min(C_w, CMAX);
    Kh = a.ckv + (int64_t)row0_w * a.ldkv + a.koff + h * 64;
    Vh = Kh + d;
#pragma unroll
    for (int t = 0; t < NTILE; t++)
#pragma unroll
      for (int i = 0; i < SL; i++) {
        const int key = min(t * KT + rg + 32 * i, C - 1);
        kv[t][i] = gld4(Kh + (key * a.ldkv + c4));
      }
  };
  {
    const int c = tid < d ? tid : 0;
    const float* pp = a.pend + (int64_t)r * d + c;
    const int64_t plane = (int64_t)a.S * d;
    if constexpr (PS) {
#if !defined(WB_PS_DRY)
      if (!ps.known_dead) {
        load_weights();
        load_keys();
      }
#endif
      if (!ps_wait(ps)) return false;
      dead = ps.known_dead ? 1 : ld_i<true>(ps.dead + r);
      if (r >= n_live || dead) { ps.saw_dead = true; return true; }
      const Buf16 xgb(a.g_x_in), pgb(a.g_pend);
      const uint32_t pvo = (uint32_t)(r * d + c);
      const int iplane = a.S * d;
      ps_nap<4>();
      constexpr int FP = 8;
      float v = 0.f, accp = gld(a.pbias + c);
      unsigned sweeps = 0;
      Gran gx{0u, 0.f}, g[FP];
#pragma unroll
      for (int j = 0; j < FP; j++) g[j] = Gran{0u, 0.f};
      for (;;) {
        if (gx.tag != ps.tag_in) gx = ld_gran(xgb, pvo, 0u);
#pragma unroll
        for (int j = 0; j < FP; j++)
          if (j < a.KSp && g[j].tag != ps.tag_in) g[j] = ld_gran(pgb, pvo, (uint32_t)(j * iplane));
        bool ok = gx.tag == ps.tag_in;
#pragma unroll
        for (int j = 0; j < FP; j++) ok &= (j >= a.KSp) || g[j].tag == ps.tag_in;
        if (ok) {
#pragma unroll
          for (int j = 0; j < FP; j++) accp += (j < a.KSp) ? g[j].v : 0.f;
          v = gx.v + accp;
          break;
        }
        if (ps_sweep_retry(sweeps, ps)) { *ps.lds_flag = 0; break; }
      }
      xfold = v;
      if (tid < d) hs[tid] = v;
    } else {
    float v = a.x_in[(int64_t)r * d + c];
    constexpr int FP = 16;
    float t[FP];
    float accp = 0.f;
    if (a.KSp > 0) {
      accp = gld(a.pbias + c);
#pragma unroll
      for (int j = 0; j < FP; j++) t[j] = pp[(int64_t)min(j, a.KSp - 1) * plane];
    }
    load_weights();
    if (r >= n_live || dead) return true;
    if (a.KSp > 0) {
#pragma unroll
      for (int j = 0; j < FP; j++) accp += (j < a.KSp) ? t[j] : 0.f;
      for (int sp = FP; sp < a.KSp; sp += FP) {
#pragma unroll
        for (int j = 0; j < FP; j++) t[j] = pp[(int64_t)min(sp + j, a.KSp - 1) * plane];
#pragma unroll
        for (int j = 0; j < FP; j++) accp += (sp + j < a.KSp) ? t[j] : 0.f;
      }
      v += accp;
    }
    xfold = v;
    if (tid < d) hs[tid] = v;
    }
  }
  if constexpr (!PS) qbias = tid < 64 ? a.bq[h * 64 + tid] : 0.f;
  if constexpr (!PS) load_keys();
  if constexpr (PS) ps_stamp(ps, 2);
  __syncthreads();
  if constexpr (PS) { if (!ps_sweeps_ok(ps)) return false; }
#if defined(WB_PS_DRY)
  if constexpr (PS) {
    if (tid < d / 4) { const Buf16 pgo(a.g_P); st_gran4(pgo, (uint32_t)((h * a.S + r) * d + tid * 4), ps.tag_out, make_float4(0.f, 0.f, 0.f, 0.f)); }
    if (h == 0 && tid < d) { const Buf16 xgo(a.g_x_out); st_gran(xgo, (uint32_t)(r * d + tid), ps.tag_out, xfold); }
    return true;
  }
#endif
  float xn_own;
  {
    float mean, denom;
    ln_stats_lds<DPL>(hs, d, lane, a.ln_eps, a.ln_inside, mean, denom);
    xn_own = (hs[own_col] - mean) / denom * g_own + b_own;
  }
  if constexpr (PS) ps_stamp_fine(ps, 4);
  {
    float acc[4] = {0.f, 0.f, 0.f, 0.f};
    const int q4 = lane >> 4;
#pragma unroll
    for (int i = 0; i < NWQ; i++) {
      const float xv = lane_get(xn_own, 4 * i + q4);
      acc[0] += xv * wqr[i].x; acc[1] += xv * wqr[i].y; acc[2] += xv * wqr[i].z; acc[3] += xv * wqr[i].w;
    }
#pragma unroll
    for (int c = 0; c < 4; c++) { acc[c] = xor16_sum(acc[c]); acc[c] = xor32_sum(acc[c]); }
    if (lane < 16) *reinterpret_cast<float4*>(&red[wave][c4]) = make_float4(acc[0], acc[1], acc[2], acc[3]);
  }
  __syncthreads();
  if constexpr (PS) ps_stamp_fine(ps, 5);
  const int cf = tid % CF, jg = tid / CF;
  const bool p5 = jg < G;
  const int jb = (p5 ? jg : 0) * RPG;
  float4 wo[RPG];
  {
    const float* wp = a.Wo + (int64_t)(h * 64 + jb) * d + cf * 4;
#pragma unroll
    for (int i = 0; i < RPG; i++) wo[i] = ld_w4(wp + (int64_t)i * d);
  }
  if (tid < 64) {
    float v = 0.f;
#pragma unroll
    for (int w8 = 0; w8 < 8; w8++) v += red[w8][tid];
    qv[tid] = (v + qbias) * a.scale;
  }
  __syncthreads();
  if constexpr (PS) ps_stamp(ps, 3);
  {
    const float4 q4 = *reinterpret_cast<const float4*>(&qv[c4]);
#pragma unroll
    for (int p = 0; p < NP; p++) {
      const float* nxt = p + 1 < NP ? Kh + (p + 1) * PASS_C * a.ldkv : Vh;
      int rgp = rg;
      if constexpr (NP > 1) WB_LAUNDER_V(rgp);
#pragma unroll
      for (int t = 0; t < NTILE; t++) {
        if constexpr (NP > 1) __builtin_amdgcn_sched_barrier(0);
#pragma unroll
        for (int i = 0; i < SL; i++) {
          const int k0 = t * KT + rgp + 32 * i, key = p * PASS_C + k0;
          float s = q4.x * kv[t][i].x + q4.y * kv[t][i].y + q4.z * kv[t][i].z + q4.w * kv[t][i].w;
          s += dpp_f<DPP_QUAD_XOR1, 0xF>(0.f, s);
          s += dpp_f<DPP_QUAD_XOR2, 0xF>(0.f, s);
          s += dpp_f<DPP_ROW_HALF_MIRROR, 0xF>(0.f, s);
          s += dpp_f<DPP_ROW_MIRROR, 0xF>(0.f, s);
          if ((tid & 15) == 0 && key < C) sc[key] = s;
          const int lim = p + 1 < NP ? max(C - 1 - (p + 1) * PASS_C, -(p + 1) * PASS_C) : C - 1;
          kv[t][i] = gld4(nxt + (min(k0, lim) * a.ldkv + c4));
        }
      }
    }
  }
  __syncthreads();
  if constexpr (PS) ps_stamp(ps, 4);
  float m = -INFINITY;
  for (int j = lane; j < C; j += 64) m = fmaxf(m, sc[j]);
  m = wave_max(m);
  float l = 0.f;
  for (int j = lane; j < C; j += 64) l += expf(sc[j] - m);
  l = wave_sum(l);
  for (int j = tid; j < C; j += NT) pbuf[j] = expf(sc[j] - m);
  __syncthreads();
  {
    float4 o = make_float4(0.f, 0.f, 0.f, 0.f);
#pragma unroll
    for (int p = 0; p < NP; p++) {
      int rgp = rg;
      if constexpr (NP > 1) WB_LAUNDER_V(rgp);
#pragma unroll
      for (int t = 0; t < NTILE; t++) {
        if constexpr (NP > 1) WB_PIN_F4(o);
#pragma unroll
        for (int i = 0; i < SL; i++) {
          const int k0 = t * KT + rgp + 32 * i, key = p * PASS_C + k0;
          const float pk = key < C ? pbuf[key] : 0.f;
          o.x += pk * kv[t][i].x; o.y += pk * kv[t][i].y; o.z += pk * kv[t][i].z; o.w += pk * kv[t][i].w;
          if (p + 1 < NP)
            kv[t][i] = gld4(Vh + (min(key + PASS_C, C - 1) * a.ldkv + c4));
        }
      }
    }
    *reinterpret_cast<float4*>(&part[rg][c4]) = o;
  }
  __syncthreads();
  if (tid < 64) {
    float v = 0.f;
#pragma unroll
    for (int g2 = 0; g2 < 32; g2++) v += part[g2][tid];
    att[tid] = v / l;
  }
  __syncthreads();
  if constexpr (PS) ps_stamp(ps, 5);
  float ov[4] = {0.f, 0.f, 0.f, 0.f};
#pragma unroll
  for (int i = 0; i < RPG; i++) {
    const float av = att[jb + i];
    ov[0] += av * wo[i].x; ov[1] += av * wo[i].y; ov[2] += av * wo[i].z; ov[3] += av * wo[i].w;
  }
  if (p5 && jg > 0) *reinterpret_cast<float4*>(&obuf[(jg - 1) * d + cf * 4]) = make_float4(ov[0], ov[1], ov[2], ov[3]);
  __syncthreads();
  if (jg == 0) {
#pragma unroll
    for (int g2 = 1; g2 < G; g2++) {
      const float4 t = *reinterpret_cast<const float4*>(&obuf[(g2 - 1) * d + cf * 4]);
      ov[0] += t.x; ov[1] += t.y; ov[2] += t.z; ov[3] += t.w;
    }
    if constexpr (PS) {
      const Buf16 pgo(a.g_P);
      st_gran4(pgo, (uint32_t)((h * a.S + r) * d + cf * 4), ps.tag_out, make_float4(ov[0], ov[1], ov[2], ov[3]));
    } else {
      *reinterpret_cast<float4*>(&a.P[((int64_t)h * a.S + r) * d + cf * 4]) = make_float4(ov[0], ov[1], ov[2], ov[3]);
    }
  }
  if (h == 0 && tid < d) {
    if constexpr (PS) { const Buf16 xgo(a.g_x_out); st_gran(xgo, (uint32_t)(r * d + tid), ps.tag_out, xfold); }
    else a.x_out[(int64_t)r * d + tid] = xfold;
  }
  return true;
}


}
}
```

### whisper-burn_amd/csrc/decode_persist.hip

```cpp
#include <hip/hip_runtime.h>

#include <climits>
#include <vector>

#include "decode.h"
#include "decode_fused_bodies.h"
#include "handoff.h"
#include "wave_ops.h"

namespace wb {
namespace {

using namespace fused;

constexpr int PS_NT = 512;
constexpr int PS_CT = 128;
constexpr int PS_NGO = 16;

template <int DPL>
__device__ __forceinline__ bool ps_finln_role(const PersistArgs& a, const int r, const PsStep& ps) {
  constexpr int d = 64 * DPL, FP = 4 * DPL;
  __shared__ __attribute__((aligned(16))) float hs[d];
  const int tid = role_tid<true>(), lane = tid & 63, wave = tid >> 6;
  const int c = tid < d ? tid : 0;
  const float g_own = a.ln_g[c], b_own = a.ln_b[c];
  float accp = a.b2_last[c];
  if (!ps_wait(ps)) return false;
  if (ld_i<true>(ps.dead + r) != 0) return true;
  ps_nap<2>();
  const Buf16 xgb(a.x_fin), pgb(a.P2);
  const uint32_t pvo = (uint32_t)(r * d + c);
  const int iplane = a.S * d;
  float v = 0.f;
  unsigned sweeps = 0;
  Gran gx{0u, 0.f}, g[FP];
#pragma unroll
  for (int j = 0; j < FP; j++) g[j] = Gran{0u, 0.f};
  for (;;) {
    if (gx.tag != ps.tag_in) gx = ld_gran(xgb, pvo, 0u);
#pragma unroll
    for (int j = 0; j < FP; j++)
      if (j < a.nb_mlp && g[j].tag != ps.tag_in) g[j] = ld_gran(pgb, pvo, (uint32_t)(j * iplane));
    bool ok = gx.tag == ps.tag_in;
#pragma unroll
    for (int j = 0; j < FP; j++) ok &= (j >= a.nb_mlp) || g[j].tag == ps.tag_in;
    if (ok) {
#pragma unroll
      for (int j = 0; j < FP; j++) accp += (j < a.nb_mlp) ? g[j].v : 0.f;
      v = gx.v + accp;
      break;
    }
    if (ps_sweep_retry(sweeps, ps)) { *ps.lds_flag = 0; break; }
  }
  if (tid < d) hs[tid] = v;
  ps_stamp(ps, 2);
  __syncthreads();
  if (!ps_sweeps_ok(ps)) return false;
  if (wave < DPL) {
    float mean, denom;
    ln_stats_lds<DPL>(hs, d, lane, a.ln_eps, a.ln_inside, mean, denom);
    const Buf16 xo(a.g_xn);
    st_gran(xo, (uint32_t)(r * d + tid), ps.tag_out, (v - mean) / denom * g_own + b_own);
  }
  return true;
}

template <int MR, int DPL>
__device__ __forceinline__ bool ps_logits_role(const PersistArgs& a, const int tile0, const int n_t, const PsStep& ps,
                                               const bool forced) {
  constexpr int d = 64 * DPL, NT = PS_NT, CT = PS_CT;
  constexpr int NR = d / 16;
  constexpr int EPT = (MR * d + NT - 1) / NT;
  constexpr int PCH = EPT <= 3 ? 8 : EPT <= 6 ? 4 : 2;
  constexpr int NQ = MR * CT / NT;
  constexpr bool TWO = DPL <= 6;
  __shared__ __attribute__((aligned(16))) float xs[MR][d];
  __shared__ __attribute__((aligned(16))) float red[8][MR][CT];
  __shared__ float tilev[MR][CT];
  const int tid = role_tid<true>(), lane = tid & 63, wave = tid >> 6;
  const int hh = lane >> 5, c4 = (lane & 31) * 4;
  const Buf16 etb(a.Et);
  auto load_tile = [&](float4 (&w)[NR], int tile) {
    const int n0 = tile * CT;
    const bool col_ok = n0 + c4 < a.vocab_ld;
    const uint32_t vo = (uint32_t)((2 * wave + hh) * NR * a.vocab_ld + n0 + (col_ok ? c4 : 0));
#pragma unroll
    for (int i = 0; i < NR; i++) w[i] = ld_f4_plain(etb, vo, (uint32_t)(i * a.vocab_ld));
  };
  float4 w0[NR], w1[TWO ? NR : 1];
  if (!forced) {
#if !defined(WB_PS_DRY)
    load_tile(w0, tile0);
    if constexpr (TWO) { if (n_t > 1) load_tile(w1, tile0 + 1); }
#endif
  }
  const int use_mask = (ps.step + 1 <= a.mask_until_len) ? 1 : 0;
  int deadm = 0;
  if (!ps_wait(ps)) return false;
  {
    int off[EPT];
#pragma unroll
    for (int i = 0; i < EPT; i++) {
      int e = tid + NT * i;
      if (e >= MR * d) e = tid;
      off[i] = e;
    }
#pragma unroll
    for (int r = 0; r < MR; r++)
      if (r >= ps.n_rows || ld_i<true>(ps.dead + min(r, ps.n_rows - 1)) != 0) deadm |= 1 << r;
    const Buf16 xgb(a.g_xn);
    float v[EPT];
    unsigned sweeps = 0;
    for (;;) {
      Gran gx[EPT];
#pragma unroll
      for (int i = 0; i < EPT; i++) gx[i] = ld_gran(xgb, (uint32_t)off[i], 0u);
      bool ok = true;
#pragma unroll
      for (int i = 0; i < EPT; i++) ok &= ((deadm >> (off[i] / d)) & 1) != 0 || gx[i].tag == ps.tag_in;
      if (ok) {
#pragma unroll
        for (int i = 0; i < EPT; i++) v[i] = ((deadm >> (off[i] / d)) & 1) ? 0.f : gx[i].v;
        break;
      }
      if (ps_sweep_retry(sweeps, ps)) { *ps.lds_flag = 0; break; }
    }
#pragma unroll
    for (int i = 0; i < EPT; i++) {
      const int e = tid + NT * i;
      if (e < MR * d) (&xs[0][0])[e] = v[i];
    }
  }
  ps_stamp(ps, 2);
  __syncthreads();
  if (!ps_sweeps_ok(ps)) return false;
  ps_stamp(ps, 3);
  if (forced) return true;
#if defined(WB_PS_DRY)
  for (int t = 0; t < n_t; t++)
    if (wave < MR && !((deadm >> wave) & 1) && lane == 0) {
      float* ts = a.tstats + ((int64_t)wave * a.n_tiles + tile0 + t) * 2;
      st_f<true>(ts, 0.f);
      st_f<true>(ts + 1, __int_as_float((tile0 + t) * CT));
    }
  return true;
#endif
  auto run_tile = [&](const float4 (&w)[NR], int tile) {
    const int n0 = tile * CT;
    float mk[NQ];
#pragma unroll
    for (int q = 0; q < NQ; q++) {
      const int col = n0 + ((tid + NT * q) & (CT - 1));
      mk[q] = (use_mask && col < a.V) ? a.mask[col] : 0.f;
    }
    float acc[MR][4];
#pragma unroll
    for (int r = 0; r < MR; r++) { acc[r][0] = acc[r][1] = acc[r][2] = acc[r][3] = 0.f; }
#pragma unroll
    for (int r = 0; r < MR; r++) {
      if ((deadm >> r) & 1) continue;
#pragma unroll
      for (int i4 = 0; i4 < NR; i4 += 4) {
        const float4 xv = *reinterpret_cast<const float4*>(&xs[r][(2 * wave + hh) * NR + i4]);
        acc[r][0] += xv.x * w[i4].x; acc[r][1] += xv.x * w[i4].y; acc[r][2] += xv.x * w[i4].z; acc[r][3] += xv.x * w[i4].w;
        acc[r][0] += xv.y * w[i4 + 1].x; acc[r][1] += xv.y * w[i4 + 1].y; acc[r][2] += xv.y * w[i4 + 1].z; acc[r][3] += xv.y * w[i4 + 1].w;
        acc[r][0] += xv.z * w[i4 + 2].x; acc[r][1] += xv.z * w[i4 + 2].y; acc[r][2] += xv.z * w[i4 + 2].z; acc[r][3] += xv.z * w[i4 + 2].w;
        acc[r][0] += xv.w * w[i4 + 3].x; acc[r][1] += xv.w * w[i4 + 3].y; acc[r][2] += xv.w * w[i4 + 3].z; acc[r][3] += xv.w * w[i4 + 3].w;
      }
    }
#pragma unroll
    for (int r = 0; r < MR; r++)
#pragma unroll
      for (int c = 0; c < 4; c++) acc[r][c] = xor32_sum(acc[r][c]);
    __syncthreads();
    if (hh == 0) {
#pragma unroll
      for (int r = 0; r < MR; r++)
        *reinterpret_cast<float4*>(&red[wave][r][c4]) = make_float4(acc[r][0], acc[r][1], acc[r][2], acc[r][3]);
    }
    __syncthreads();
#pragma unroll
    for (int q = 0; q < NQ; q++) {
      const int e = tid + NT * q, r = e / CT, c = e & (CT - 1);
      float v = 0.f;
#pragma unroll
      for (int w8 = 0; w8 < 8; w8++) v += red[w8][r][c];
      v += mk[q];
      if (n0 + c >= a.V) v = -INFINITY;
      tilev[r][c] = v;
    }
    __syncthreads();
    if (wave < MR && !((deadm >> wave) & 1)) {
      const int r = wave;
      const float v0 = tilev[r][lane], v1 = tilev[r][lane + 64];
      float bvv; int bi;
      if (better(v0, lane, v1, lane + 64)) { bvv = v0; bi = lane; } else { bvv = v1; bi = lane + 64; }
      wave_argmax(bvv, bi);
      if (lane == 0) {
        float* ts = a.tstats + ((int64_t)r * a.n_tiles + tile) * 2;
        st_f<true>(ts, bvv);
        st_f<true>(ts + 1, __int_as_float(n0 + bi));
      }
    }
  };
  run_tile(w0, tile0);
  ps_stamp(ps, 4);
  if constexpr (TWO) {
    if (n_t > 1) run_tile(w1, tile0 + 1);
    ps_stamp(ps, 5);
    for (int t = 2; t < n_t; t++) { load_tile(w0, tile0 + t); run_tile(w0, tile0 + t); }
  } else {
    for (int t = 1; t < n_t; t++) { load_tile(w0, tile0 + t); run_tile(w0, tile0 + t); }
  }
  return true;
}

__device__ __forceinline__ bool ps_merge_role(const PersistArgs& a, const int r, const int e, const PsStep& ps0,
                                              const unsigned* clog, const int* n_per_ctr) {
  __shared__ float redv[8];
  __shared__ int redi[8];
  const int tid = role_tid<true>(), lane = tid & 63, wave = tid >> 6;
  const PsStep& ps = ps0;
  {
    __shared__ unsigned tgt[8];
    if (tid < 8) tgt[tid] = (unsigned)(e + 1) * (unsigned)n_per_ctr[tid];
    __syncthreads();
    if (!hx_wait_many(clog, tgt, 8, ps.ctl, ps.step, 1000, ps.lds_flag)) return false;
  }
  ps_stamp(ps, 1);
  const int len = ps.step + 1;
  const int fin_now = ld_i<true>(a.dead + r);
  const int tok_prev = ld_i<true>(a.gctl + GC_HDR + r);
  int gi;
  if (e < a.n_forced) {
    gi = a.forced[e];
  } else {
    float bv = -INFINITY; int bi = 0x7fffffff;
    for (int t = tid; t < a.n_tiles; t += PS_NT) {
      const float* ts = a.tstats + ((int64_t)r * a.n_tiles + t) * 2;
      const float v = ld_f<true>(ts);
      const int id = __float_as_int(ld_f<true>(ts + 1));
      if (better(v, id, bv, bi)) { bv = v; bi = id; }
    }
    wave_argmax(bv, bi);
    if (lane == 0) { redv[wave] = bv; redi[wave] = bi; }
    __syncthreads();
    float gv = redv[0]; gi = redi[0];
#pragma unroll
    for (int j = 1; j < 8; j++)
      if (better(redv[j], redi[j], gv, gi)) { gv = redv[j]; gi = redi[j]; }
    if ((unsigned)gi >= 0x7fffffffu) { gi = a.eot; if (tid == 0) a.gctl[GC_BAD] = 1; }
  }
  const int finished = fin_now || (gi == a.eot && e >= a.n_forced);
  const int tok_next = fin_now ? tok_prev : gi;
  if (tid == 0 && !fin_now) {
    st_i_sc1(a.gctl + GC_HDR + r, gi);
    a.gtok[r * a.Lmax + len] = gi;
    a.gctl[GC_HDR + 2 * a.S + r] = len + 1;
    if (gi == a.eot && e >= a.n_forced) {
      a.gctl[GC_HDR + a.S + r] = 1;
      st_i_sc1(a.dead + r, 1);
      const unsigned n = __hip_atomic_fetch_add(reinterpret_cast<unsigned*>(a.ctl + HX_NDONE), 1u, __ATOMIC_RELAXED,
                                                __HIP_MEMORY_SCOPE_AGENT) + 1u;
      if ((int)n == ps.n_rows) st_i_sc1(a.ctl + HX_STOP, ps.step + 1);
    }
  }
  if (tid == 0 && r == 0) a.gctl[GC_STEP] = ps.step + 1;
  if (len < a.Lmax) {
    const Buf16 xb(a.x0);
    const float4* ev = reinterpret_cast<const float4*>(a.E + (int64_t)tok_next * a.d);
    const float4* pp = reinterpret_cast<const float4*>(a.pos + (int64_t)len * a.d);
    const unsigned tag_x = a.tag_base + 1u + 3u * (unsigned)((e + 1) * a.n_layer);
    for (int c = tid; c < (a.d >> 2); c += PS_NT) {
      const float4 x = ev[c], y = pp[c];
      st_gran4(xb, (uint32_t)(r * a.d + 4 * c), tag_x, make_float4(x.x + y.x, x.y + y.y, x.z + y.z, x.w + y.w));
    }
    const int nstep = ps.step + 1;
    int* tab_new = a.tabs + (size_t)(nstep & 1) * a.S * a.Lmax;
    for (int p = tid; p <= len; p += PS_NT) tab_new[r * a.Lmax + p] = p * a.S + r;
  }
  (void)finished;
  return true;
}

template <int DPL, int MR, int NP>
__global__ __launch_bounds__(PS_NT) void dec_persist_kernel(PersistArgs a) {
  __shared__ int wait_flag;
  const int NL = a.n_layer, S = a.S, R = a.n_rows, H = a.n_head, NB = a.nb_mlp;
  auto cptr = [&](int c) { return reinterpret_cast<unsigned*>(a.ctl + HX_HDR + c * HX_LINE); };
  const int C_X = 0, C_ATTN = S, C_CROSS = S + NL * S, C_MLP = C_CROSS + NL, C_LOG = C_MLP + NL, C_GO = C_LOG + 8;
  int n_per_ctr[8];
#pragma unroll
  for (int k = 0; k < 8; k++) n_per_ctr[k] = (a.n_logits_roles + 7 - k) / 8;
  const int i_lo = a.role_off[blockIdx.x], i_hi = a.role_off[blockIdx.x + 1];
  unsigned long long dead_seen = 0;
  for (int e = 0; e < a.n_steps; e++) {
    for (int i = i_lo; i < i_hi; i++) {
      const PsRole role = a.roles[i];
      PsStep ps;
      ps.known_dead = i - i_lo < 64 && ((dead_seen >> (i - i_lo)) & 1ull) != 0;
      ps.ctl = a.ctl; ps.step = a.step0 + e; ps.n_rows = R; ps.dead = a.dead; ps.lds_flag = &wait_flag;
      unsigned long long* stp = a.stamps ? a.stamps + ((size_t)e * a.n_roles + i) * PS_STAMPS : nullptr;
      if (stp && threadIdx.x == 0) stp[0] = wall_clock64();
      ps.stamp = stp;
      int out;
      bool ok;
      const unsigned tag_l = a.tag_base + 2u + 3u * (unsigned)(e * NL + (role.kind <= PSR_MLP ? role.layer : NL - 1));
      if (role.kind == PSR_ATTN) {
        const AttnFusedArgs la = a.layers[role.layer].attn;
        if (role.layer == 0) { ps.ctr_index = C_X + role.b; ps.target = (unsigned)e; }
        else { ps.ctr_index = C_CROSS + role.layer - 1; ps.target = (unsigned)(e + 1) * H * R; }
        ps.ctr = cptr(ps.ctr_index);
        ps.tag_out = tag_l; ps.tag_in = tag_l - 1u;
        ok = dec_attn_body<DPL, true>(la, role.a, role.b, ps);
        out = C_ATTN + role.layer * S + role.b;
      } else if (role.kind == PSR_CROSS) {
        const CrossFusedArgs la = a.layers[role.layer].cross;
        if (role.layer == 0) { ps.ctr_index = C_X + role.b; ps.target = (unsigned)e; }
        else { ps.ctr_index = C_MLP + role.layer - 1; ps.target = (unsigned)(e + 1) * NB; }
        ps.ctr = cptr(ps.ctr_index);
        ps.tag_out = tag_l + 1u; ps.tag_in = tag_l;
        ok = dec_cross_body<DPL, true, NP>(la, role.a, role.b, ps);
        out = C_CROSS + role.layer;
      } else if (role.kind == PSR_MLP) {
        const MlpFusedArgs la = a.layers[role.layer].mlp;
        ps.ctr_index = C_ATTN + role.layer * S; ps.target = (unsigned)(e + 1) * H; ps.n_ctr = R;
        ps.ctr = cptr(ps.ctr_index);
        ps.tag_out = tag_l + 2u; ps.tag_in = tag_l + 1u;
        ok = dec_mlp_body<MR, DPL, false, true>(la, role.a, ps);
        out = C_MLP + role.layer;
      } else if (role.kind == PSR_FINLN) {
        ps.ctr_index = C_CROSS + NL - 1; ps.target = (unsigned)(e + 1) * H * R;
        ps.ctr = cptr(ps.ctr_index);
        ps.tag_in = tag_l + 2u; ps.tag_out = tag_l + 2u;
        ok = ps_finln_role<DPL>(a, role.b, ps);
        out = C_GO + PS_NGO;
      } else if (role.kind == PSR_LOGITS) {
        ps.ctr_index = C_GO + (role.layer % PS_NGO); ps.target = (unsigned)(e + 1);
        ps.ctr = cptr(ps.ctr_index);
        ps.tag_in = tag_l + 2u;
        ok = ps_logits_role<MR, DPL>(a, role.a, role.b, ps, e < a.n_forced);
        out = C_LOG + (role.layer & 7);
      } else {
        ok = ps_merge_role(a, role.b, e, ps, cptr(C_LOG), n_per_ctr);
        out = C_X + role.b;
      }
      if (!ok) return;
      if (ps.saw_dead && i - i_lo < 64) dead_seen |= 1ull << (i - i_lo);
      if (stp && threadIdx.x == 0) stp[6] = wall_clock64();
      if (role.kind == PSR_CROSS && role.layer == NL - 1)
        hx_arrive_broadcast(cptr(out), (unsigned)(e + 1) * H * R, cptr(C_GO), PS_NGO, (unsigned)(e + 1));
      else
        hx_arrive(cptr(out));
      if (stp && threadIdx.x == 0) stp[7] = wall_clock64();
    }
  }
}

__global__ void ps_seed_kernel(const float* __restrict__ x, int n, void* gx, unsigned tag) {
  const Buf16 b(gx);
  for (int i = blockIdx.x * blockDim.x + threadIdx.x; i < n; i += gridDim.x * blockDim.x) st_gran(b, (uint32_t)i, tag, x[i]);
}

template <int DPL, int MR, int NP>
int max_blocks_per_cu() {
  int nb = 0;
  if (hipOccupancyMaxActiveBlocksPerMultiprocessor(&nb, (dec_persist_kernel<DPL, MR, NP>), PS_NT, 0) != hipSuccess) return 0;
  return nb;
}

}

int ps_ctl_ints(int S, int n_layer) { return HX_HDR + (S + n_layer * S + 2 * n_layer + 8 + PS_NGO + 1) * HX_LINE; }

bool dec_persist_supported(int d, int n_rows, int max_keys) {
  if (n_rows < 1 || n_rows > 8) return false;
  if (max_keys > CROSS_FUSED_MAX_PASSES * CROSS_FUSED_MAX_C) return false;
  if (max_keys > CROSS_FUSED_MAX_C && n_rows > 4) return false;
  if (d == 128 || d == 384) return true;
  return d == 512 && n_rows <= 4;
}

int dec_persist_max_grid(int device, int d, int n_rows, int max_keys) {
  if (!dec_persist_supported(d, n_rows, max_keys)) return 0;
  int cus = 0, coop = 0;
  if (hipDeviceGetAttribute(&coop, hipDeviceAttributeCooperativeLaunch, device) != hipSuccess || !coop) return 0;
  if (hipDeviceGetAttribute(&cus, hipDeviceAttributeMultiprocessorCount, device) != hipSuccess || cus <= 0) return 0;
  int per = 0;
  const bool big = n_rows > 4;
  if (max_keys > CROSS_FUSED_MAX_C)
    per = d == 128 ? max_blocks_per_cu<2, 4, 2>() : d == 384 ? max_blocks_per_cu<6, 4, 2>() : max_blocks_per_cu<8, 4, 2>();
  else if (d == 128) per = big ? max_blocks_per_cu<2, 8, 1>() : max_blocks_per_cu<2, 4, 1>();
  else if (d == 384) per = big ? max_blocks_per_cu<6, 8, 1>() : max_blocks_per_cu<6, 4, 1>();
  else per = max_blocks_per_cu<8, 4, 1>();
  if (per <= 0) return 0;
  return cus * 1;
}

void launch_ps_seed(hipStream_t st, const float* x, int n, void* gx, unsigned tag) {
  hipLaunchKernelGGL(ps_seed_kernel, dim3((n + 255) / 256), dim3(256), 0, st, x, n, gx, tag);
}

int launch_dec_persist(hipStream_t st, const PersistArgs& a, int grid) {
  const dim3 g(grid), b(PS_NT);
  const bool big = a.n_rows > 4;
  hipError_t e = hipErrorInvalidValue;
#define WB_PS(DPL_, MR_, NP_) e = WB_LAUNCH_COOP((dec_persist_kernel<DPL_, MR_, NP_>), g, b, 0, st, a)
  if (a.n_pass > 1) {
    if (big) return -1;
    if (a.d == 128) WB_PS(2, 4, 2); else if (a.d == 384) WB_PS(6, 4, 2); else if (a.d == 512) WB_PS(8, 4, 2);
  }
  else if (a.d == 128) { if (big) WB_PS(2, 8, 1); else WB_PS(2, 4, 1); }
  else if (a.d == 384) { if (big) WB_PS(6, 8, 1); else WB_PS(6, 4, 1); }
  else if (a.d == 512 && !big) WB_PS(8, 4, 1);
#undef WB_PS
  return e == hipSuccess ? 0 : -1;
}

}
```

### whisper-burn_amd/csrc/switches.h

```cpp
#pragma once

namespace wb {
namespace sw {

enum Kind { DEFAULT_ON, OPT_IN, UNSET_OR_1, TRI, INT, STR };

#define WB_BOOL_SWITCHES(X)                                                                                                          \
  X(graph, "WHISPER_HIP_GRAPH", DEFAULT_ON, "on", "replay captured hipGraphs of the decode steps; 0: enqueue every step eagerly")    \
  X(chain, "WHISPER_HIP_CHAIN", DEFAULT_ON, "on", "device-chained greedy decode; 0: one host round trip per step")                   \
  X(beam_chain, "WHISPER_HIP_BEAM_CHAIN", DEFAULT_ON, "on", "beam bookkeeping on the device; 0: host-driven beam search")            \
  X(persist, "WHISPER_HIP_PERSIST", DEFAULT_ON, "on", "persistent flag-chained greedy kernel; 0: one launch per sublayer")           \
  X(persist_prefill, "WHISPER_HIP_PERSIST_PREFILL", DEFAULT_ON, "on", "the persistent launch runs the prompt itself; 0: host prefill") \
  X(poll, "WHISPER_HIP_POLL", DEFAULT_ON, "on", "chained greedy: spin on mapped progress flags; 0: copy + synchronise per chunk")    \
  X(speculate, "WHISPER_HIP_SPECULATE", OPT_IN, "off", "chained greedy: enqueue one segment ahead of the finished flags")            \
  X(fuse_sub, "WHISPER_HIP_FUSE_SUB", DEFAULT_ON, "on", "fused self-attention and MLP sublayer kernels; 0: per-matrix GEMVs")        \
  X(fuse_x, "WHISPER_HIP_FUSE_X", DEFAULT_ON, "on", "fused cross-attention sublayer kernel; 0: chunked cross-attention + GEMV")      \
  X(fuse_q, "WHISPER_HIP_FUSE_Q", DEFAULT_ON, "on", "chunked cross-attention blocks project their own queries")                      \
  X(fuse_co, "WHISPER_HIP_FUSE_CO", OPT_IN, "off", "chunked cross-attention blocks apply the out-projection too")                    \
  X(fuse16, "WHISPER_HIP_FUSE16", DEFAULT_ON, "on", "9 - 16 live rows stay on the fused sublayer kernels; 0: batch mode")            \
  X(batch_skinny, "WHISPER_HIP_BATCH_SKINNY", DEFAULT_ON, "on", "batch mode: skinny weight-stream GEMM up to 64 rows; 0: tiled GEMM") \
  X(cross_stream, "WHISPER_HIP_CROSS_STREAM", DEFAULT_ON, "on", "batch mode, one beam per window: streaming cross-attention")        \
  X(sk_pair, "WHISPER_HIP_SK_PAIR", OPT_IN, "off", "skinny GEMM: the waves' partial tiles meet pairwise")                            \
  X(mlp16_mfma, "WHISPER_HIP_MLP16_MFMA", DEFAULT_ON, "on", "9 - 16-row fused MLP on the matrix cores; 0: two row groups of 8")      \
  X(logits_mfma, "WHISPER_HIP_LOGITS_MFMA", DEFAULT_ON, "on", "9 - 16-row logits product on the matrix cores")                       \
  X(logits_preln, "WHISPER_HIP_LOGITS_PRELN", DEFAULT_ON, "on", "9 - 16-row logits: fold + LayerNorm once, in its own launch")       \
  X(logits_mr16, "WHISPER_HIP_LOGITS_MR16", DEFAULT_ON, "on", "9 - 16-row logits GEMV as one 16-row tile")                           \
  X(encoder_split, "WHISPER_HIP_ENCODER_SPLIT", UNSET_OR_1, "on", "split-precision (fp16 hi / lo) encoder-side GEMMs; 0: exact f32") \
  X(decoder_split, "WHISPER_HIP_DECODER_SPLIT", DEFAULT_ON, "on", "split-precision batch-mode decoder GEMM; 0: exact f32")           \
  X(encoder_pieces, "WHISPER_HIP_ENCODER_PIECES", DEFAULT_ON, "on", "encoder activations travel as fp16 pieces between split GEMMs") \
  X(attn_f16, "WHISPER_HIP_ATTN_F16", DEFAULT_ON, "on", "encoder attention on fp16 pieces; 0: the f32 kernels")                      \
  X(attn_kvsplit, "WHISPER_HIP_ATTN_KVSPLIT", DEFAULT_ON, "on", "encoder attention splits long key ranges across blocks")            \
  X(gpu_turn, "WHISPER_HIP_GPU_TURN", DEFAULT_ON, "on", "one entry point at a time per device and process (developer: 0 drops it)")  \
  X(session_pool, "WHISPER_HIP_SESSION_POOL", DEFAULT_ON, "on", "released sessions are parked for reuse; 0: freed (developer A/B)")  \
  X(pcm_stage, "WHISPER_HIP_PCM_STAGE", OPT_IN, "off", "host PCM is uploaded through a pinned per-session buffer")
#define WB_INT_SWITCHES(X)                                                                                                           \
  X(cross_stream_fuse, "WHISPER_HIP_CROSS_STREAM_FUSE", TRI, -1, "streaming cross-attention folds / projects its query; unset: d <= 768") \
  X(sk_max_blocks, "WHISPER_HIP_SK_MAX_BLOCKS", INT, 256, "skinny GEMM: most blocks a K-split may launch")                           \
  X(split_tile, "WHISPER_HIP_SPLIT_TILE", INT, 0, "split-precision GEMM: force a tile shape (developer A/B; 0: choose)")             \
  X(enc_trace_extra, "WHISPER_HIP_ENC_TRACE_EXTRA", INT, 0, "bit mask of extra stages in the encoder trace (1 pcm, 2 mel, 4 maxima)")
#define WB_STR_SWITCHES(X)                                                                                                           \
  X(enc_trace, "WHISPER_HIP_ENC_TRACE", STR, nullptr, "directory for per-thread dumps of the encoder stages (developer)")            \
  X(ps_stamps, "WHISPER_HIP_PS_STAMPS", STR, nullptr, "file for the persistent kernel's role timeline (developer)")                  \
  X(persist_inject_fail, "WHISPER_HIP_PERSIST_INJECT_FAIL", STR, nullptr, "test hook: \"launch\" = the cooperative launch is refused")

#define WB_SW_DECL(fn, name, kind, dflt, what) bool fn();
WB_BOOL_SWITCHES(WB_SW_DECL)
#undef WB_SW_DECL
#define WB_SW_DECL(fn, name, kind, dflt, what) int fn();
WB_INT_SWITCHES(WB_SW_DECL)
#undef WB_SW_DECL
#define WB_SW_DECL(fn, name, kind, dflt, what) const char* fn();
WB_STR_SWITCHES(WB_SW_DECL)
#undef WB_SW_DECL

}
}
```

Baseline: 2178 x real-time.

## Keep step-invariant attention/cross weights resident in LDS in the persistent decode kernel

Each persistent-kernel block that owns a single attention or cross-attention role preloads part of its QKV/Wo weights (and cross key/value tiles) into an LDS arena once, instead of re-streaming them from global memory every decode step. To make room, the per-role shared buffers are moved into structs and unioned into one arena, with the leftover space used for resident slots. The added LDS use may lower occupancy or change scheduling, and the path is on by default with an env switch to disable or log it.

```diff
diff --git a/whisper-burn_amd/csrc/decode.h b/whisper-burn_amd/csrc/decode.h
--- a/whisper-burn_amd/csrc/decode.h
+++ b/whisper-burn_amd/csrc/decode.h
@@ -201,6 +201,7 @@
   const PsLayerArgs* layers = nullptr;
   const PsRole* roles = nullptr; int n_roles = 0;
   const int* role_off = nullptr;
+  const int* res_role = nullptr;
   int n_logits_roles = 0;
   int n_layer = 0, n_rows = 0, S = 0, d = 0, n_head = 0, nb_mlp = 0;
   int n_pass = 1;
@@ -221,6 +222,7 @@
 };
 int ps_ctl_ints(int S, int n_layer);
 bool dec_persist_supported(int d, int n_rows, int max_keys);
+int dec_persist_resident_slots(int d, int n_rows, int max_keys);
 int dec_persist_max_grid(int device, int d, int n_rows, int max_keys);
 int launch_dec_persist(hipStream_t st, const PersistArgs& a, int grid);
 void launch_ps_seed(hipStream_t st, const float* x, int n, void* gx, unsigned tag);
diff --git a/whisper-burn_amd/csrc/decode_chain.cpp b/whisper-burn_amd/csrc/decode_chain.cpp
--- a/whisper-burn_amd/csrc/decode_chain.cpp
+++ b/whisper-burn_amd/csrc/decode_chain.cpp
@@ -111,9 +111,21 @@
     roles.insert(roles.end(), deal[b].begin(), deal[b].end());
   }
   role_off[grid] = (int)roles.size();
+  const char* res_sw = sw::persist_resident();
+  const bool res_on = !(res_sw && res_sw[0] == '0') && dec_persist_resident_slots(d, W, s->maxC) > 0;
+  std::vector<int> res_role(grid, -1);
+  int n_res = 0;
+  if (res_on)
+    for (int b = 0; b < grid; b++) {
+      int n_layer_roles = 0, at = -1;
+      for (int i = role_off[b]; i < role_off[b + 1]; i++)
+        if (roles[i].kind <= PSR_MLP) { n_layer_roles++; at = i; }
+      if (n_layer_roles == 1 && roles[at].kind != PSR_MLP) { res_role[b] = at; n_res++; }
+    }
+  if (res_sw && !strcmp(res_sw, "log")) fprintf(stderr, "persist resident blocks: %d of %d\n", n_res, grid);
   const int n_ctl = ps_ctl_ints(S, NL);
   WB_TRY(s->ps_layers.ensure(la.size() * sizeof(PsLayerArgs)));
-  WB_TRY(s->ps_roles.ensure(roles.size() * sizeof(PsRole) + role_off.size() * 4));
+  WB_TRY(s->ps_roles.ensure(roles.size() * sizeof(PsRole) + (role_off.size() + res_role.size()) * 4));
   WB_TRY(s->ps_ctl.ensure((size_t)n_ctl * 4));
   WB_TRY(s->ps_dead.ensure((size_t)S * 4));
   WB_TRY(s->ps_tstats.ensure((size_t)S * n_tiles * 2 * 4));
@@ -121,6 +133,8 @@
   ctl0[HX_STOP] = INT_MAX;
   WB_HIP(hipMemcpyAsync(s->ps_layers.p, la.data(), la.size() * sizeof(PsLayerArgs), hipMemcpyHostToDevice, st));
   WB_HIP(hipMemcpyAsync(s->ps_roles.p, roles.data(), roles.size() * sizeof(PsRole), hipMemcpyHostToDevice, st));
+  WB_HIP(hipMemcpyAsync(static_cast<char*>(s->ps_roles.p) + roles.size() * sizeof(PsRole) + role_off.size() * 4, res_role.data(),
+                        res_role.size() * 4, hipMemcpyHostToDevice, st));
   WB_HIP(hipMemcpyAsync(static_cast<char*>(s->ps_roles.p) + roles.size() * sizeof(PsRole), role_off.data(), role_off.size() * 4,
                         hipMemcpyHostToDevice, st));
   WB_HIP(hipMemcpyAsync(s->ps_ctl.p, ctl0.data(), (size_t)n_ctl * 4, hipMemcpyHostToDevice, st));
@@ -128,6 +142,7 @@
   PersistArgs a;
   a.layers = s->ps_layers.as<PsLayerArgs>(); a.roles = s->ps_roles.as<PsRole>(); a.n_roles = (int)roles.size();
   a.role_off = reinterpret_cast<const int*>(static_cast<char*>(s->ps_roles.p) + roles.size() * sizeof(PsRole));
+  if (n_res > 0) a.res_role = a.role_off + role_off.size();
   a.n_logits_roles = n_lg;
   a.n_layer = NL; a.n_rows = W; a.S = S; a.d = d; a.n_head = H; a.nb_mlp = NB;
   a.n_pass = s->maxC > CROSS_FUSED_MAX_C ? 2 : 1;
diff --git a/whisper-burn_amd/csrc/decode_fused.hip b/whisper-burn_amd/csrc/decode_fused.hip
--- a/whisper-burn_amd/csrc/decode_fused.hip
+++ b/whisper-burn_amd/csrc/decode_fused.hip
@@ -20,15 +20,18 @@
     a.row0 = r0; a.x_in += sh; a.x_out += sh; a.P += sh;
     if (a.pend) a.pend += sh;
   }
-  dec_mlp_body<MR, DPL, REC, false>(a, blockIdx.x, PsStep());
+  __shared__ MlpLds<MR, DPL, REC> sm;
+  dec_mlp_body<MR, DPL, REC, false>(a, blockIdx.x, PsStep(), sm);
 }
 template <int DPL>
 __global__ __launch_bounds__(512) void dec_attn_fused_kernel(AttnFusedArgs a) {
-  dec_attn_body<DPL, false>(a, blockIdx.x, blockIdx.y, PsStep());
+  __shared__ AttnLds<DPL> sm;
+  dec_attn_body<DPL, false>(a, blockIdx.x, blockIdx.y, PsStep(), sm);
 }
 template <int DPL, int NP>
 __global__ __launch_bounds__(512) void dec_cross_fused_kernel(CrossFusedArgs a) {
-  dec_cross_body<DPL, false, NP>(a, blockIdx.x, blockIdx.y, PsStep());
+  __shared__ CrossLds<DPL, NP> sm;
+  dec_cross_body<DPL, false, NP>(a, blockIdx.x, blockIdx.y, PsStep(), sm);
 }
 
 
diff --git a/whisper-burn_amd/csrc/decode_fused_bodies.h b/whisper-burn_amd/csrc/decode_fused_bodies.h
--- a/whisper-burn_amd/csrc/decode_fused_bodies.h
+++ b/whisper-burn_amd/csrc/decode_fused_bodies.h
@@ -63,9 +63,9 @@
 }
 
 #ifdef WB_STAMPS
-#define WB_STAMP_DECL __shared__ unsigned long long stamp_buf[16]
-#define WB_STAMP(i) do { if (threadIdx.x == 0 && blockIdx.x == 0 && blockIdx.y == 0) stamp_buf[i] = wall_clock64(); } while (0)
-#define WB_STAMP_FLUSH(a, n) do { if (threadIdx.x == 0 && blockIdx.x == 0 && blockIdx.y == 0 && (a).stamps) for (int _i = 0; _i < (n); _i++) (a).stamps[_i] = stamp_buf[_i]; } while (0)
+#define WB_STAMP_DECL unsigned long long stamp_buf[16];
+#define WB_STAMP(i) do { if (threadIdx.x == 0 && blockIdx.x == 0 && blockIdx.y == 0) sm.stamp_buf[i] = wall_clock64(); } while (0)
+#define WB_STAMP_FLUSH(a, n) do { if (threadIdx.x == 0 && blockIdx.x == 0 && blockIdx.y == 0 && (a).stamps) for (int _i = 0; _i < (n); _i++) (a).stamps[_i] = sm.stamp_buf[_i]; } while (0)
 #else
 #define WB_STAMP_DECL
 #define WB_STAMP(i) do {} while (0)
@@ -74,6 +74,61 @@
 
 constexpr int FD_MAX = 512;
 constexpr int FA_MAXPOS = 448;
+
+
+constexpr int ROLE_NT = 512;
+template <int MR, int DPL, bool REC>
+struct MlpLds {
+  static constexpr int d = 64 * DPL, HS = 64, G = d / 4 <= 32 ? 8 : 4;
+  alignas(16) float hs[MR][d];
+  alignas(16) float red[8][MR][HS];
+  alignas(16) float hid[MR][HS];
+  alignas(16) float obuf[(G - 1) * MR * d];
+  float mlb[REC ? MR : 1][48][2];
+  float coef[REC ? MR : 1][48];
+  WB_STAMP_DECL
+};
+template <int DPL>
+struct AttnLds {
+  static constexpr int d = 64 * DPL, G = d / 4 <= 32 ? 8 : 4;
+  static constexpr int RED = (8 * 192 > (G - 1) * d) ? 8 * 192 : (G - 1) * d;
+  alignas(16) float hs[d];
+  alignas(16) float red[RED];
+  alignas(16) float qkv[192];
+  int tbs[FA_MAXPOS];
+  float sc[FA_MAXPOS];
+  alignas(16) float part[32][64];
+  alignas(16) float att[64];
+  WB_STAMP_DECL
+};
+template <int DPL, int NP>
+struct CrossLds {
+  static constexpr int d = 64 * DPL, G = d / 4 <= 32 ? 8 : 4, CMAX = NP * CROSS_FUSED_MAX_C;
+  alignas(16) float hs[d];
+  alignas(16) float red[8][64];
+  alignas(16) float qv[64];
+  float sc[CMAX];
+  float pbuf[CMAX];
+  alignas(16) float part[32][64];
+  alignas(16) float att[64];
+  alignas(16) float obuf[(G - 1) * d];
+};
+
+template <int DPL, int NP, int RS>
+struct ResGeom {
+  static constexpr int d = 64 * DPL, G = d / 4 <= 32 ? 8 : 4, RPG = 64 / G;
+  static constexpr int KW = d / 8, RK = DPL >= 6 ? 8 : 16, NIT = KW / RK;
+  static constexpr int NRND = (NIT - 2 < RS / RK ? NIT - 2 : RS / RK) > 0 ? (NIT - 2 < RS / RK ? NIT - 2 : RS / RK) : 0;
+  static constexpr int WO_A = NRND * RK;
+  static constexpr int NWO_A = RS - WO_A < RPG ? RS - WO_A : RPG;
+  static constexpr int SL = 4, NTILE = CROSS_FUSED_MAX_C / 128;
+  static constexpr int NVT = NP > 1 ? 0 : (RS / SL < NTILE ? RS / SL : NTILE);
+  static constexpr int WO_X = NVT * SL;
+  static constexpr int NWO_X = NP > 1 ? 0 : (RS - WO_X < RPG ? RS - WO_X : RPG);
+  static_assert(RS >= 0 && WO_A + NWO_A <= RS && WO_X + NWO_X <= RS, "resident slots");
+};
+__device__ __forceinline__ float4 res_ld(const float4* res, int slot, int tid) { return res[slot * ROLE_NT + tid]; }
+__device__ __forceinline__ void res_st(float4* res, int slot, int tid, const float4& v) { res[slot * ROLE_NT + tid] = v; }
 
 __device__ __forceinline__ float gelu_erf_f(float x) {
   return 0.5f * x * (1.0f + erff(x * 0.70710678118654752440f));
@@ -206,7 +261,7 @@
 __device__ __forceinline__ float lane_get(float v, int src) { return __shfl(v, src, 64); }
 
 template <int MR, int DPL, bool REC, bool PS>
-__device__ __forceinline__ bool dec_mlp_body(const MlpFusedArgs& a, const int jblk, const PsStep& ps) {
+__device__ __forceinline__ bool dec_mlp_body(const MlpFusedArgs& a, const int jblk, const PsStep& ps, MlpLds<MR, DPL, REC>& sm) {
   constexpr int HS = 64, NT = 512;
   constexpr int d = 64 * DPL;
   constexpr int CF = d / 4;
@@ -214,13 +269,8 @@
   constexpr int RPG = HS / G;
   constexpr int EPT = (MR * d + NT - 1) / NT;
   constexpr int PCH = EPT <= 3 ? 8 : EPT <= 6 ? 6 : 3;
-  __shared__ __attribute__((aligned(16))) float hs[MR][d];
-  __shared__ __attribute__((aligned(16))) float red[8][MR][HS];
-  __shared__ __attribute__((aligned(16))) float hid[MR][HS];
-  __shared__ __attribute__((aligned(16))) float obuf[(G - 1) * MR * d];
-  __shared__ float mlb[REC ? MR : 1][48][2];
-  __shared__ float coef[REC ? MR : 1][48];
-  WB_STAMP_DECL;
+  static_assert(G == MlpLds<MR, DPL, REC>::G, "LDS struct geometry");
+  auto& hs = sm.hs; auto& red = sm.red; auto& hid = sm.hid; auto& obuf = sm.obuf; auto& mlb = sm.mlb; auto& coef = sm.coef;
   WB_STAMP(0);
   const int tid = role_tid<PS>(), lane = tid & 63, wave = tid >> 6;
   const int j0 = jblk * HS;
@@ -543,8 +593,9 @@
   return true;
 }
 
-template <int DPL, bool PS>
-__device__ __forceinline__ bool dec_attn_body(const AttnFusedArgs& a, const int h, const int r, const PsStep& ps) {
+template <int DPL, bool PS, int RS = 0>
+__device__ __forceinline__ bool dec_attn_body(const AttnFusedArgs& a, const int h, const int r, const PsStep& ps, AttnLds<DPL>& sm,
+                                              const float4* res = nullptr) {
   constexpr int NT = 512;
   constexpr int d = 64 * DPL;
   constexpr int KW = d / 8;
@@ -553,16 +604,10 @@
   constexpr int CF = d / 4;
   constexpr int G = CF <= 32 ? 8 : 4;
   constexpr int RPG = 64 / G;
-  constexpr int RED = (8 * 192 > (G - 1) * d) ? 8 * 192 : (G - 1) * d;
   constexpr int PT = 128, PSL = PT * 16 / NT;
-  __shared__ __attribute__((aligned(16))) float hs[d];
-  __shared__ __attribute__((aligned(16))) float red[RED];
-  __shared__ __attribute__((aligned(16))) float qkv[192];
-  __shared__ int tbs[FA_MAXPOS];
-  __shared__ float sc[FA_MAXPOS];
-  __shared__ __attribute__((aligned(16))) float part[32][64];
-  __shared__ __attribute__((aligned(16))) float att[64];
-  WB_STAMP_DECL;
+  using RG = ResGeom<DPL, 1, PS ? RS : 0>;
+  static_assert(G == AttnLds<DPL>::G && RG::RK == RK && RG::NIT == NIT && RG::RPG == RPG && NT == ROLE_NT, "LDS struct / resident geometry");
+  auto& hs = sm.hs; auto& red = sm.red; auto& qkv = sm.qkv; auto& tbs = sm.tbs; auto& sc = sm.sc; auto& part = sm.part; auto& att = sm.att;
   WB_STAMP(0);
   const int tid = role_tid<PS>(), lane = tid & 63, wave = tid >> 6;
   if (h >= a.n_head) return true;
@@ -708,19 +753,37 @@
   }
   if constexpr (PS) ps_stamp_fine(ps, 4);
   WB_STAMP(2);
+  const int nres = (RG::NRND > 0 && res != nullptr) ? RG::NRND : 0;
+  const int nreg = NIT - nres;
   float acc[4] = {0.f, 0.f, 0.f, 0.f};
 #pragma unroll 1
-  for (int it = 0; it < NIT; it += 2) {
+  for (int n = 0; n < nreg; n += 2) {
 #pragma unroll
     for (int b = 0; b < 2; b++) {
-      if (it + b < NIT) {
-        const int kb = RK * (it + b);
+      if (n + b < nreg) {
+        const int kb = RK * (n + b < 2 ? n + b : n + b + nres);
 #pragma unroll
         for (int j = 0; j < RK; j++) {
           const float xv = __int_as_float(__builtin_amdgcn_readlane(__float_as_int(xn_own), kb + j));
           acc[0] += xv * wr[b][j].x; acc[1] += xv * wr[b][j].y; acc[2] += xv * wr[b][j].z; acc[3] += xv * wr[b][j].w;
         }
-        if (it + b + 2 < NIT) load_round(wr[b], it + b + 2);
+        if (n + b + 2 < nreg) load_round(wr[b], n + b + 2 + nres);
+      }
+      if constexpr (RG::NRND > 0) {
+        if (b == 1 && n == 0 && nres > 0) {
+#pragma unroll 1
+          for (int q = 0; q < RG::NRND; q++) {
+            float4 wl[RK];
+#pragma unroll
+            for (int j = 0; j < RK; j++) wl[j] = res_ld(res, q * RK + j, tid);
+            const int kb = RK * (2 + q);
+#pragma unroll
+            for (int j = 0; j < RK; j++) {
+              const float xv = __int_as_float(__builtin_amdgcn_readlane(__float_as_int(xn_own), kb + j));
+              acc[0] += xv * wl[j].x; acc[1] += xv * wl[j].y; acc[2] += xv * wl[j].z; acc[3] += xv * wl[j].w;
+            }
+          }
+        }
       }
     }
   }
@@ -733,8 +796,12 @@
   float4 wo[RPG];
   {
     const float* wp = a.Wo + (int64_t)(h * 64 + jb) * d + cf * 4;
-#pragma unroll
-    for (int i = 0; i < RPG; i++) wo[i] = ld_w4(wp + (int64_t)i * d);
+    if (RG::NWO_A == 0 || res == nullptr) {
+#pragma unroll
+      for (int i = 0; i < RG::NWO_A; i++) wo[i] = ld_w4(wp + (int64_t)i * d);
+    }
+#pragma unroll
+    for (int i = RG::NWO_A; i < RPG; i++) wo[i] = ld_w4(wp + (int64_t)i * d);
   }
   if (seg_ok) *reinterpret_cast<float4*>(&red[wave * 192 + seg * 64 + c4]) = make_float4(acc[0], acc[1], acc[2], acc[3]);
   __syncthreads();
@@ -832,6 +899,12 @@
   __syncthreads();
   WB_STAMP(6);
   if constexpr (PS) ps_stamp(ps, 5);
+  if constexpr (RG::NWO_A > 0) {
+    if (res != nullptr) {
+#pragma unroll
+      for (int i = 0; i < RG::NWO_A; i++) wo[i] = res_ld(res, RG::WO_A + i, tid);
+    }
+  }
   float ov[4] = {0.f, 0.f, 0.f, 0.f};
 #pragma unroll
   for (int i = 0; i < RPG; i++) {
@@ -867,8 +940,36 @@
   return true;
 }
 
-template <int DPL, bool PS, int NP = 1>
-__device__ __forceinline__ bool dec_cross_body(const CrossFusedArgs& a, const int h, const int r, const PsStep& ps) {
+template <int DPL, int RS>
+__device__ __forceinline__ void dec_attn_res_fill(const AttnFusedArgs& a, const int h, float4* res) {
+  using RG = ResGeom<DPL, 1, RS>;
+  constexpr int d = 64 * DPL, KW = d / 8, RK = RG::RK, CF = d / 4, G = RG::G, RPG = RG::RPG;
+  const int tid = role_tid<true>(), lane = tid & 63, wave = tid >> 6;
+  const int seg = lane >> 4, c4 = (lane & 15) * 4;
+  const float* wq = a.Wqkv + (int64_t)(wave * KW) * a.ldqkv + (seg < 3 ? seg : 0) * d + h * 64 + c4;
+#pragma unroll 1
+  for (int q = 0; q < RG::NRND; q++) {
+    float4 w[RK];
+#pragma unroll
+    for (int j = 0; j < RK; j++) w[j] = ld_w4(wq + (int64_t)(RK * (2 + q) + j) * a.ldqkv);
+#pragma unroll
+    for (int j = 0; j < RK; j++) res_st(res, q * RK + j, tid, w[j]);
+  }
+  if constexpr (RG::NWO_A > 0) {
+    const int cf = tid % CF, jg = tid / CF;
+    const int jb = (jg < G ? jg : 0) * RPG;
+    const float* wp = a.Wo + (int64_t)(h * 64 + jb) * d + cf * 4;
+    float4 w[RG::NWO_A];
+#pragma unroll
+    for (int i = 0; i < RG::NWO_A; i++) w[i] = ld_w4(wp + (int64_t)i * d);
+#pragma unroll
+    for (int i = 0; i < RG::NWO_A; i++) res_st(res, RG::WO_A + i, tid, w[i]);
+  }
+}
+
+template <int DPL, bool PS, int NP = 1, int RS = 0>
+__device__ __forceinline__ bool dec_cross_body(const CrossFusedArgs& a, const int h, const int r, const PsStep& ps,
+                                               CrossLds<DPL, NP>& sm, const float4* res = nullptr) {
   constexpr int NT = 512;
   constexpr int PASS_C = CROSS_FUSED_MAX_C, CMAX = NP * PASS_C;
   constexpr int d = 64 * DPL;
@@ -878,14 +979,12 @@
   constexpr int RPG = 64 / G;
   constexpr int KT = 128, NTILE = CROSS_FUSED_MAX_C / KT, SL = KT * 16 / NT;
   static_assert(CROSS_FUSED_MAX_C % KT == 0 && SL * NT == KT * 16, "tile geometry");
-  __shared__ __attribute__((aligned(16))) float hs[d];
-  __shared__ __attribute__((aligned(16))) float red[8][64];
-  __shared__ __attribute__((aligned(16))) float qv[64];
-  __shared__ float sc[CMAX];
-  __shared__ float pbuf[CMAX];
-  __shared__ __attribute__((aligned(16))) float part[32][64];
-  __shared__ __attribute__((aligned(16))) float att[64];
-  __shared__ __attribute__((aligned(16))) float obuf[(G - 1) * d];
+  using RG = ResGeom<DPL, NP, PS ? RS : 0>;
+  static_assert(G == CrossLds<DPL, NP>::G && CMAX == CrossLds<DPL, NP>::CMAX && RG::SL == SL && RG::NTILE == NTILE && RG::RPG == RPG &&
+                NT == ROLE_NT, "LDS struct / resident geometry");
+  auto& hs = sm.hs; auto& red = sm.red; auto& qv = sm.qv; auto& sc = sm.sc; auto& pbuf = sm.pbuf; auto& part = sm.part; auto& att = sm.att;
+  auto& obuf = sm.obuf;
+  const bool res_v = RG::NVT > 0 && res != nullptr;
   const int tid = role_tid<PS>(), lane = tid & 63, wave = tid >> 6;
   if (h >= a.n_head) return true;
   int n_live, w_row, dead;
@@ -1040,8 +1139,12 @@
   float4 wo[RPG];
   {
     const float* wp = a.Wo + (int64_t)(h * 64 + jb) * d + cf * 4;
-#pragma unroll
-    for (int i = 0; i < RPG; i++) wo[i] = ld_w4(wp + (int64_t)i * d);
+    if (RG::NWO_X == 0 || res == nullptr) {
+#pragma unroll
+      for (int i = 0; i < RG::NWO_X; i++) wo[i] = ld_w4(wp + (int64_t)i * d);
+    }
+#pragma unroll
+    for (int i = RG::NWO_X; i < RPG; i++) wo[i] = ld_w4(wp + (int64_t)i * d);
   }
   if (tid < 64) {
     float v = 0.f;
@@ -1071,7 +1174,7 @@
           s += dpp_f<DPP_ROW_MIRROR, 0xF>(0.f, s);
           if ((tid & 15) == 0 && key < C) sc[key] = s;
           const int lim = p + 1 < NP ? max(C - 1 - (p + 1) * PASS_C, -(p + 1) * PASS_C) : C - 1;
-          kv[t][i] = gld4(nxt + (min(k0, lim) * a.ldkv + c4));
+          if (t >= RG::NVT || !res_v) kv[t][i] = gld4(nxt + (min(k0, lim) * a.ldkv + c4));
         }
       }
     }
@@ -1099,6 +1202,7 @@
         for (int i = 0; i < SL; i++) {
           const int k0 = t * KT + rgp + 32 * i, key = p * PASS_C + k0;
           const float pk = key < C ? pbuf[key] : 0.f;
+          if (t < RG::NVT) { if (res_v) kv[t][i] = res_ld(res, t * SL + i, tid); }
           o.x += pk * kv[t][i].x; o.y += pk * kv[t][i].y; o.z += pk * kv[t][i].z; o.w += pk * kv[t][i].w;
           if (p + 1 < NP)
             kv[t][i] = gld4(Vh + (min(key + PASS_C, C - 1) * a.ldkv + c4));
@@ -1116,6 +1220,12 @@
   }
   __syncthreads();
   if constexpr (PS) ps_stamp(ps, 5);
+  if constexpr (RG::NWO_X > 0) {
+    if (res != nullptr) {
+#pragma unroll
+      for (int i = 0; i < RG::NWO_X; i++) wo[i] = res_ld(res, RG::WO_X + i, tid);
+    }
+  }
   float ov[4] = {0.f, 0.f, 0.f, 0.f};
 #pragma unroll
   for (int i = 0; i < RPG; i++) {
@@ -1144,6 +1254,36 @@
   return true;
 }
 
-
-}
-}
+template <int DPL, int NP, int RS>
+__device__ __forceinline__ void dec_cross_res_fill(const CrossFusedArgs& a, const int h, const int r, float4* res) {
+  using RG = ResGeom<DPL, NP, RS>;
+  constexpr int d = 64 * DPL, CF = d / 4, G = RG::G, RPG = RG::RPG, KT = 128, SL = RG::SL;
+  const int tid = role_tid<true>();
+  const int rg = tid >> 4, c4 = (tid & 15) * 4;
+  if constexpr (RG::NVT > 0) {
+    const int C = min(gld(a.win_C + r), CROSS_FUSED_MAX_C), row0 = gld(a.win_row0 + r);
+    const float* Vh = a.ckv + (int64_t)row0 * a.ldkv + a.koff + h * 64 + d;
+#pragma unroll 1
+    for (int t = 0; t < RG::NVT; t++) {
+      float4 v[SL];
+#pragma unroll
+      for (int i = 0; i < SL; i++) v[i] = gld4(Vh + (min(t * KT + rg + 32 * i, C - 1) * a.ldkv + c4));
+#pragma unroll
+      for (int i = 0; i < SL; i++) res_st(res, t * SL + i, tid, v[i]);
+    }
+  }
+  if constexpr (RG::NWO_X > 0) {
+    const int cf = tid % CF, jg = tid / CF;
+    const int jb = (jg < G ? jg : 0) * RPG;
+    const float* wp = a.Wo + (int64_t)(h * 64 + jb) * d + cf * 4;
+    float4 w[RG::NWO_X];
+#pragma unroll
+    for (int i = 0; i < RG::NWO_X; i++) w[i] = ld_w4(wp + (int64_t)i * d);
+#pragma unroll
+    for (int i = 0; i < RG::NWO_X; i++) res_st(res, RG::WO_X + i, tid, w[i]);
+  }
+}
+
+
+}
+}
diff --git a/whisper-burn_amd/csrc/decode_persist.hip b/whisper-burn_amd/csrc/decode_persist.hip
--- a/whisper-burn_amd/csrc/decode_persist.hip
+++ b/whisper-burn_amd/csrc/decode_persist.hip
@@ -18,9 +18,11 @@
 constexpr int PS_NGO = 16;
 
 template <int DPL>
-__device__ __forceinline__ bool ps_finln_role(const PersistArgs& a, const int r, const PsStep& ps) {
+struct FinLnLds { alignas(16) float hs[64 * DPL]; };
+template <int DPL>
+__device__ __forceinline__ bool ps_finln_role(const PersistArgs& a, const int r, const PsStep& ps, FinLnLds<DPL>& sm) {
   constexpr int d = 64 * DPL, FP = 4 * DPL;
-  __shared__ __attribute__((aligned(16))) float hs[d];
+  auto& hs = sm.hs;
   const int tid = role_tid<true>(), lane = tid & 63, wave = tid >> 6;
   const int c = tid < d ? tid : 0;
   const float g_own = a.ln_g[c], b_own = a.ln_b[c];
@@ -66,17 +68,21 @@
 }
 
 template <int MR, int DPL>
+struct LogitsLds {
+  alignas(16) float xs[MR][64 * DPL];
+  alignas(16) float red[8][MR][PS_CT];
+  float tilev[MR][PS_CT];
+};
+template <int MR, int DPL>
 __device__ __forceinline__ bool ps_logits_role(const PersistArgs& a, const int tile0, const int n_t, const PsStep& ps,
-                                               const bool forced) {
+                                               const bool forced, LogitsLds<MR, DPL>& sm) {
   constexpr int d = 64 * DPL, NT = PS_NT, CT = PS_CT;
   constexpr int NR = d / 16;
   constexpr int EPT = (MR * d + NT - 1) / NT;
   constexpr int PCH = EPT <= 3 ? 8 : EPT <= 6 ? 4 : 2;
   constexpr int NQ = MR * CT / NT;
   constexpr bool TWO = DPL <= 6;
-  __shared__ __attribute__((aligned(16))) float xs[MR][d];
-  __shared__ __attribute__((aligned(16))) float red[8][MR][CT];
-  __shared__ float tilev[MR][CT];
+  auto& xs = sm.xs; auto& red = sm.red; auto& tilev = sm.tilev;
   const int tid = role_tid<true>(), lane = tid & 63, wave = tid >> 6;
   const int hh = lane >> 5, c4 = (lane & 31) * 4;
   const Buf16 etb(a.Et);
@@ -215,14 +221,14 @@
   return true;
 }
 
+struct MergeLds { float redv[8]; int redi[8]; unsigned tgt[8]; };
 __device__ __forceinline__ bool ps_merge_role(const PersistArgs& a, const int r, const int e, const PsStep& ps0,
-                                              const unsigned* clog, const int* n_per_ctr) {
-  __shared__ float redv[8];
-  __shared__ int redi[8];
+                                              const unsigned* clog, const int* n_per_ctr, MergeLds& sm) {
+  auto& redv = sm.redv; auto& redi = sm.redi;
   const int tid = role_tid<true>(), lane = tid & 63, wave = tid >> 6;
   const PsStep& ps = ps0;
   {
-    __shared__ unsigned tgt[8];
+    auto& tgt = sm.tgt;
     if (tid < 8) tgt[tid] = (unsigned)(e + 1) * (unsigned)n_per_ctr[tid];
     __syncthreads();
     if (!hx_wait_many(clog, tgt, 8, ps.ctl, ps.step, 1000, ps.lds_flag)) return false;
@@ -284,8 +290,37 @@
 }
 
 template <int DPL, int MR, int NP>
+union PsRoleLds {
+  MlpLds<MR, DPL, false> mlp; AttnLds<DPL> attn; CrossLds<DPL, NP> cross;
+  FinLnLds<DPL> finln; LogitsLds<MR, DPL> logits; MergeLds merge;
+};
+constexpr int PS_LDS_BYTES = 160 * 1024;
+constexpr bool ps_resident_instance(int DPL, int MR, int NP) { return !(DPL >= 6 && (MR == 8 || NP == 2)); }
+template <int DPL, int MR, int NP>
+struct PsArena {
+  static constexpr int ROLE_BYTES = (int)((sizeof(PsRoleLds<DPL, MR, NP>) + 15) / 16 * 16);
+  static constexpr int FLAG_BYTES = 16;
+  static constexpr int RS = ps_resident_instance(DPL, MR, NP) ? (PS_LDS_BYTES - ROLE_BYTES - FLAG_BYTES) / (PS_NT * 16) : 0;
+  static constexpr int BYTES = ROLE_BYTES + FLAG_BYTES + RS * PS_NT * 16;
+  static_assert(RS >= 0 && BYTES <= PS_LDS_BYTES, "the persistent kernel's LDS arena exceeds 160 KB");
+  static constexpr bool USEFUL = ResGeom<DPL, NP, RS>::WO_A + ResGeom<DPL, NP, RS>::NWO_A + ResGeom<DPL, NP, RS>::WO_X +
+                                 ResGeom<DPL, NP, RS>::NWO_X > 0;
+};
+static_assert(PS_NT == ROLE_NT, "block size");
+#define WB_PS_INSTANCES(X) X(2, 4, 1) X(2, 8, 1) X(6, 4, 1) X(6, 8, 1) X(8, 4, 1) X(2, 4, 2) X(6, 4, 2) X(8, 4, 2)
+#define WB_PS_CHECK(DPL_, MR_, NP_) static_assert(PsArena<DPL_, MR_, NP_>::BYTES <= 160 * 1024, "LDS arena of an instance");
+WB_PS_INSTANCES(WB_PS_CHECK)
+#undef WB_PS_CHECK
+
+template <int DPL, int MR, int NP>
 __global__ __launch_bounds__(PS_NT) void dec_persist_kernel(PersistArgs a) {
-  __shared__ int wait_flag;
+  using AR = PsArena<DPL, MR, NP>;
+  constexpr int RS = AR::RS;
+  __shared__ PsRoleLds<DPL, MR, NP> lds;
+  __shared__ __attribute__((aligned(16))) int wait_flag[AR::FLAG_BYTES / 4];
+  __shared__ __attribute__((aligned(16))) float4 res_buf[RS > 0 ? RS * PS_NT : 1];
+  static_assert(sizeof(lds) <= AR::ROLE_BYTES && sizeof(wait_flag) == AR::FLAG_BYTES && sizeof(res_buf) <= (RS > 0 ? RS : 1) * PS_NT * 16 &&
+                AR::BYTES + (RS > 0 ? 0 : 16) <= PS_LDS_BYTES, "the three LDS objects are what PsArena accounts for");
   const int NL = a.n_layer, S = a.S, R = a.n_rows, H = a.n_head, NB = a.nb_mlp;
   auto cptr = [&](int c) { return reinterpret_cast<unsigned*>(a.ctl + HX_HDR + c * HX_LINE); };
   const int C_X = 0, C_ATTN = S, C_CROSS = S + NL * S, C_MLP = C_CROSS + NL, C_LOG = C_MLP + NL, C_GO = C_LOG + 8;
@@ -293,13 +328,25 @@
 #pragma unroll
   for (int k = 0; k < 8; k++) n_per_ctr[k] = (a.n_logits_roles + 7 - k) / 8;
   const int i_lo = a.role_off[blockIdx.x], i_hi = a.role_off[blockIdx.x + 1];
+#if defined(WB_PS_DRY)
+  constexpr bool RES = false;
+#else
+  constexpr bool RES = RS > 0;
+#endif
+  int res_i = -1;
+  if (RES && a.res_role != nullptr) res_i = a.res_role[blockIdx.x];
+  if (res_i >= i_lo && res_i < i_hi) {
+    const PsRole role = a.roles[res_i];
+    if (role.kind == PSR_ATTN) dec_attn_res_fill<DPL, RS>(a.layers[role.layer].attn, role.a, res_buf);
+    else if (role.kind == PSR_CROSS) dec_cross_res_fill<DPL, NP, RS>(a.layers[role.layer].cross, role.a, role.b, res_buf);
+  }
   unsigned long long dead_seen = 0;
   for (int e = 0; e < a.n_steps; e++) {
     for (int i = i_lo; i < i_hi; i++) {
       const PsRole role = a.roles[i];
       PsStep ps;
       ps.known_dead = i - i_lo < 64 && ((dead_seen >> (i - i_lo)) & 1ull) != 0;
-      ps.ctl = a.ctl; ps.step = a.step0 + e; ps.n_rows = R; ps.dead = a.dead; ps.lds_flag = &wait_flag;
+      ps.ctl = a.ctl; ps.step = a.step0 + e; ps.n_rows = R; ps.dead = a.dead; ps.lds_flag = &wait_flag[0];
       unsigned long long* stp = a.stamps ? a.stamps + ((size_t)e * a.n_roles + i) * PS_STAMPS : nullptr;
       if (stp && threadIdx.x == 0) stp[0] = wall_clock64();
       ps.stamp = stp;
@@ -312,7 +359,7 @@
         else { ps.ctr_index = C_CROSS + role.layer - 1; ps.target = (unsigned)(e + 1) * H * R; }
         ps.ctr = cptr(ps.ctr_index);
         ps.tag_out = tag_l; ps.tag_in = tag_l - 1u;
-        ok = dec_attn_body<DPL, true>(la, role.a, role.b, ps);
+        ok = dec_attn_body<DPL, true, RS>(la, role.a, role.b, ps, lds.attn, i == res_i ? res_buf : nullptr);
         out = C_ATTN + role.layer * S + role.b;
       } else if (role.kind == PSR_CROSS) {
         const CrossFusedArgs la = a.layers[role.layer].cross;
@@ -320,29 +367,29 @@
         else { ps.ctr_index = C_MLP + role.layer - 1; ps.target = (unsigned)(e + 1) * NB; }
         ps.ctr = cptr(ps.ctr_index);
         ps.tag_out = tag_l + 1u; ps.tag_in = tag_l;
-        ok = dec_cross_body<DPL, true, NP>(la, role.a, role.b, ps);
+        ok = dec_cross_body<DPL, true, NP, RS>(la, role.a, role.b, ps, lds.cross, i == res_i ? res_buf : nullptr);
         out = C_CROSS + role.layer;
       } else if (role.kind == PSR_MLP) {
         const MlpFusedArgs la = a.layers[role.layer].mlp;
         ps.ctr_index = C_ATTN + role.layer * S; ps.target = (unsigned)(e + 1) * H; ps.n_ctr = R;
         ps.ctr = cptr(ps.ctr_index);
         ps.tag_out = tag_l + 2u; ps.tag_in = tag_l + 1u;
-        ok = dec_mlp_body<MR, DPL, false, true>(la, role.a, ps);
+        ok = dec_mlp_body<MR, DPL, false, true>(la, role.a, ps, lds.mlp);
         out = C_MLP + role.layer;
       } else if (role.kind == PSR_FINLN) {
         ps.ctr_index = C_CROSS + NL - 1; ps.target = (unsigned)(e + 1) * H * R;
         ps.ctr = cptr(ps.ctr_index);
         ps.tag_in = tag_l + 2u; ps.tag_out = tag_l + 2u;
-        ok = ps_finln_role<DPL>(a, role.b, ps);
+        ok = ps_finln_role<DPL>(a, role.b, ps, lds.finln);
         out = C_GO + PS_NGO;
       } else if (role.kind == PSR_LOGITS) {
         ps.ctr_index = C_GO + (role.layer % PS_NGO); ps.target = (unsigned)(e + 1);
         ps.ctr = cptr(ps.ctr_index);
         ps.tag_in = tag_l + 2u;
-        ok = ps_logits_role<MR, DPL>(a, role.a, role.b, ps, e < a.n_forced);
+        ok = ps_logits_role<MR, DPL>(a, role.a, role.b, ps, e < a.n_forced, lds.logits);
         out = C_LOG + (role.layer & 7);
       } else {
-        ok = ps_merge_role(a, role.b, e, ps, cptr(C_LOG), n_per_ctr);
+        ok = ps_merge_role(a, role.b, e, ps, cptr(C_LOG), n_per_ctr, lds.merge);
         out = C_X + role.b;
       }
       if (!ok) return;
@@ -369,6 +416,16 @@
   return nb;
 }
 
+}
+
+int dec_persist_resident_slots(int d, int n_rows, int max_keys) {
+  if (!dec_persist_supported(d, n_rows, max_keys)) return 0;
+  const int dpl = d / 64, mr = n_rows > 4 ? 8 : 4, np = max_keys > CROSS_FUSED_MAX_C ? 2 : 1;
+#define WB_PS_SLOTS(DPL_, MR_, NP_) \
+  if (dpl == DPL_ && mr == MR_ && np == NP_) return PsArena<DPL_, MR_, NP_>::USEFUL ? PsArena<DPL_, MR_, NP_>::RS : 0;
+  WB_PS_INSTANCES(WB_PS_SLOTS)
+#undef WB_PS_SLOTS
+  return 0;
 }
 
 int ps_ctl_ints(int S, int n_layer) { return HX_HDR + (S + n_layer * S + 2 * n_layer + 8 + PS_NGO + 1) * HX_LINE; }
diff --git a/whisper-burn_amd/csrc/switches.h b/whisper-burn_amd/csrc/switches.h
--- a/whisper-burn_amd/csrc/switches.h
+++ b/whisper-burn_amd/csrc/switches.h
@@ -41,6 +41,7 @@
 #define WB_STR_SWITCHES(X)                                                                                                           \
   X(enc_trace, "WHISPER_HIP_ENC_TRACE", STR, nullptr, "directory for per-thread dumps of the encoder stages (developer)")            \
   X(ps_stamps, "WHISPER_HIP_PS_STAMPS", STR, nullptr, "file for the persistent kernel's role timeline (developer)")                  \
+  X(persist_resident, "WHISPER_HIP_PERSIST_RESIDENT", STR, nullptr, "persistent kernel: step-invariant operands stay in LDS (on); 0: off; log: on + report") \
   X(persist_inject_fail, "WHISPER_HIP_PERSIST_INJECT_FAIL", STR, nullptr, "test hook: \"launch\" = the cooperative launch is refused")
 
 #define WB_SW_DECL(fn, name, kind, dflt, what) bool fn();
```

Measured after the change: 2222 x real-time, median of 6. 1.02x the previous value.
